# qingqing-zijin/LEAD-YOLO

Measured on AMD Instinct MI355X. Metric: images/sec (640x640) fwd+bwd, higher is better.
Workload: dtype bf16; 1 GPU; lead-yolo-s bs=64/gpu 3x640x640 bf16 full train step: uint8 batch -> train-mode forward (batch-statistics BN), ComputeLoss, HIP backward, clip 10, SGD-nesterov 3 groups, ModelEMA update (BASELINE.json configs[2]); random-init weights; global_batch=64, parallelism=dp1 (single GPU, no collective), world_size=1

## Files before the change

### include/lead_yolo_hip.h

```cpp
#ifndef LEAD_YOLO_HIP_H
#define LEAD_YOLO_HIP_H
#ifdef __cplusplus
extern "C" {
#endif

enum { LY_F32 = 0, LY_BF16 = 1 };
int ly_abi_version(void);
const char* ly_last_error(void);

int ly_mlpblock_fwd(const void* x , void* y , int n_img, int H, int W, int C, const void* wp, const void* w1,
                    const void* w2, const float* bn_scale, const float* bn_shift, double* stats, int dtype, void* stream);
int ly_mlpblock_pconv(const void* x , void* z , int n_img, int H, int W, int C, const void* wp, int dtype, void* stream);
int ly_mlpblock_bwd_ok(int C, int dtype);
long ly_mlpblock_bwd_slab_floats(int C);
int ly_mlpblock_bwd(const void* x , const void* dy , void* g , int n_img, int H, int W, int C, const void* wp, const void* w1,
                    const void* w2t, const void* w1t, const float* a, const float* b, const float* alpha, const float* kappa, const float* lambda,
                    double* stats, float* slab, long slab_floats, float* dw1, float* dw2, int pass, int dtype, void* stream);
int ly_mlpblock_bwd_dx_ok(int C, int W, int dtype);
int ly_mlpblock_bwd_dx(const void* g , const void* dy , const void* x , void* dx , int n_img, int H, int W, int C, const void* wpt,
                       float* slab, long slab_floats, float* dwp, int lddw, int dw_ts, int dw_cs, int dtype, void* stream);
int ly_mlpblock_hidden_tiles(int C);

enum { LY_ACT_NONE_ = 0, LY_ACT_RELU_ = 1, LY_ACT_SILU_ = 2 };
enum { LY_GATHER_ROWS = 0,
// ... 117 lines not shown
  float* dwc_part; int ng;
  int dtype;
} LyRf3cBwdParams;
int ly_rf3c_bwd(const LyRf3cBwdParams* p, int pass, void* stream);
int ly_rf3c_wgrad(const LyRf3cBwdParams* p, void* stream);


int ly_sppf_pool(const void* x , int ldx, int n_img, int H, int W, int C, int k, void* out , int ldo, int dtype, void* stream);
int ly_detect_tail(const void* y , int ldy, int n_img, int H, int W, int na, int no, const float* anchors, float stride,
                   float* p, float* z, long zrows, long zoff, int dtype, void* stream);
int ly_detect_level(const void* x , int ldx, int n_img, int H, int W, int K, const void* wp, int nat, const float* bias, int na, int no,
                    const float* anchors, float stride, float* p, float* z, long zrows, long zoff, int dtype, void* stream);
int ly_detect_level_ok(int K, int na, int no, int dtype);
int ly_detect_level_aug(const void* x , int ldx, int n_img, int H, int W, int K, const void* wp, int nat, const float* bias, int na, int no,
                        const float* anchors, float stride, float* p, float* z, long zrows, long zoff, float dscale, int dflip, float img_w,
                        int dtype, void* stream);
int ly_detect_tail_aug(const void* y , int ldy, int n_img, int H, int W, int na, int no, const float* anchors, float stride,
                       float* p, float* z, long zrows, long zoff, float dscale, int dflip, float img_w, int dtype, void* stream);

enum { LY_F16 = 2 };
#define LY_SCALE_IMG_MAX 4
typedef struct LyScaleImgSpec {
  void* out;
  int Hs, Ws;
  int Ho, Wo;
  int flip;
} LyScaleImgSpec;
int ly_scale_img(const void* x , int n_img, int C, int H, int W, const LyScaleImgSpec* specs, int nspec, float pad, int dtype, void* stream);

typedef struct LyMosaicTile {
  long off;
  int h, w;
  int x1a, y1a, x2a, y2a;
  int x1b, y1b;
  int lab, nlab;
  int src;
  int unused;
  double padw, padh;
} LyMosaicTile;
typedef struct LyMosaicImage {
  LyMosaicTile tile[4];
  double m[6];
  float minv[6];
  double scale;
  int mosaic;
  int flipud, fliplr;
  int unused;
  const unsigned char* lut;
} LyMosaicImage;
int ly_mosaic_img(const unsigned char* bank, const LyMosaicImage* imgs, int n_img, int s, unsigned char* out, void* stream);
int ly_mosaic_labels(const double* labels, const LyMosaicImage* imgs, int n_img, int s, int max_labels, float* targets, long cap, void* stream);
int ly_detect_head_bwd(const float* dp, int n_img, int H, int W, int na, int no, void* du , int ldu, float* dbias,
                       int dbias_f64 , int dtype, void* stream);


int ly_chan_moments(const void* x , int ldx, long rows, int C, double* mom , int dtype, void* stream);
int ly_coordatt_conv1_stats(const float* pool, long positions, int C, int mip, const float* w1, const float* b1,
                            double* stats , void* stream);
int ly_sum_rows_f64(const double* src, int R, int C, double* dst, void* stream);

int ly_rfcbam_tap_moments(const void* x , int ldx, int n_img, int H, int W, int C, int s, double* mom , int dtype, void* stream);
int ly_rfcbam_gen_prepare(const double* mom, int C, int k, const float* gen_w, const float* gamma, const float* beta, float eps,
                          float momentum, double count, float* running_mean, float* running_var, long* nbt, float* out8, float* a1,
                          float* wq_stats, float* wq_main, float* wq_c , int mom_stripes , void* stream);

int ly_nms_candidates(const float* pred, int bs, int N, int no, float conf_thres, unsigned long long class_mask, float* score, float* det,
                      void* stream);
int ly_nms_candidates_ml(const float* pred, int bs, int N, int no, float conf_thres, unsigned long long class_mask, float* score, float* det,
                         void* stream);
int ly_nms_greedy(const float* det, const long* order, const float* sorted_score, int bs, int N, float iou_thres, float max_wh, int max_det,
                  int max_nms, int* keep, int* count, void* stream);


int ly_bnact_fwd(const void* u , int ldu, long rows, int C, const float* a, const float* b, int act, void* y , int ldy, int dtype, void* stream);
int ly_bnact_bwd_reduce(const void* dy , int lddy, const void* u , int ldu, long rows, int C, const float* a, const float* b,
                        int act, double* sums , int dtype, void* stream);
int ly_bnact_bwd_apply(const void* dy , int lddy, const void* u , int ldu, long rows, int C, const float* a, const float* b,
                       int act, const float* alpha, const float* kappa, const float* lambda, void* du , int lddu, int dtype, void* stream);
int ly_bnact_bwd_reduce_pair(const void* dy1 , int lddy1, const void* dy2 , int lddy2, int csplit, const void* u , int ldu, long rows, int C,
                             const float* a, const float* b, int act, double* sums1, double* sums2, int dtype, void* stream);
int ly_bnact_bwd_apply_pair(const void* dy1 , int lddy1, const void* dy2 , int lddy2, int csplit, const void* u , int ldu, long rows, int C,
                            const float* a, const float* b, int act, const float* alpha, const float* kappa, const float* lambda, void* du , int lddu,
                            int dtype, void* stream);

typedef struct LyWgradParams {
  long M;
  int H, W;
  int N;
  const void* du; int lddu;
  const void* x; int ldx;
  int Hin, Win, Cin;
  int ks, stride, pad;
  int nchw, up2;
  float* dw; int lddw;
  int dtype;
  int dw_ts, dw_cs, n_valid, c_valid;
  const float* x_scale; const float* x_shift;
  float* ws; long ws_floats;
} LyWgradParams;
int ly_wgrad(const LyWgradParams* p, void* stream);
int ly_wgrad_group(const LyWgradParams* arr, int n, void* stream);
int ly_tune_wgrad3(int on);

int ly_up2_bwd(const void* d , int ldd, int n_img, int Hs, int Ws, int C, void* out , int ldo, int dtype, void* stream);
int ly_unpatch(const void* g , int n_img, int Ho, int Wo, int C, int ks, void* dx , int dtype, void* stream);
int ly_sum_rows(const float* src, long R, long C, long ld, float* dst, int accumulate, void* stream);
int ly_patch4_rows_u8(const unsigned char* img, int n_img, int C, int H, int W, void* rows , int dtype, void* stream);
int ly_patch4_wgrad_u8(const unsigned char* img, int n_img, int C, int H, int W, const void* du , int lddu, int N, float scale, float* slab,
                       long slab_floats, float* dw , int dtype, void* stream);

int ly_coordatt_gate_bwd(const void* dout , int ldd, const void* x , int ldx, int n_img, int H, int W, int C, const float* a_h,
                         const float* a_w, void* dx , int lddx, float* da_h, float* da_w, int bands, int slabs, int dtype, void* stream);
int ly_pool_hw_bwd(const float* gp, int n_img, int H, int W, int C, void* dx , int lddx, int accumulate, int dtype, void* stream);
int ly_maxpool_arg(const void* x , int ldx, int n_img, int H, int W, int C, int k, unsigned char* arg, int lda, int dtype, void* stream);
int ly_maxpool_gather(const unsigned char* arg, int lda, const float* d_up, int ldu, const void* d_own, int ldd, int own_dtype, int n_img, int H,
                      int W, int C, int k, void* out, int ldo, int out_dtype, void* stream);
int ly_sppf_bwd(const void* buf , int ldb, const void* d , int ldd, int n_img, int H, int W, int c, int k, void* out , int ldo, int dtype,
                void* stream);
int ly_mlp_dx(const void* dy , const void* g , const void* t , int ldt, long rows, int C, int c4, void* dx , int dtype, void* stream);
int ly_maxpool_bwd(const void* x , int ldx, const float* dy, int lddy, int n_img, int H, int W, int C, int k, float* dx, int lddx,
                   int dtype, void* stream);

int ly_rf_generate(const void* x , int ldx, int n_img, int H, int W, int C, int k, int s, const float* wg, void* ug , int dtype, void* stream);
int ly_rf_bwd_attn(int n_img, int H, int W, int C, int k, int s, const void* ug , const void* dcd , const float* ag, const float* bg,
                   const float* ca, const float* rfa, void* cd , float* d_rfa, float* gmax, float* d_ca, int dtype, void* stream);
int ly_rfa_bwd(const float* d_rfa, const float* rfa, const float* mm, const float* w18, int n_img, int Hk, int Wk, float* d_mm,
               float* dw18, int dw18_f64 , void* stream);
int ly_rf_bwd_relu(int n_img, int H, int W, int C, int k, int s, const void* ug , void* dcd , const float* ag, const float* bg,
                   const float* ca, const float* rfa, const float* gmax, const float* d_mm, float* sums, int dtype, void* stream);
int ly_rf_bwd_gen(const void* x , int ldx, int n_img, int H, int W, int C, int k, int s, const void* ug , void* dv , const float* alpha,
                  const float* kappa, const float* lambda, float* dwg, int part_rows, int dtype, void* stream);
int ly_rf_bwd_dx(int n_img, int H, int W, int C, int k, int s, const void* dug , const float* wg, void* dx , int lddx,
                 const float* addnc , float add_scale,
                 int dtype, void* stream);
int ly_se_bwd(const float* part, int slices, int n_img, int HW, int C, const float* wa, const float* wb, int R, const float* ca,
              const void* d_ca , int d_ca_f64, float* dwa, float* dwb,
              float* dgap, float* ws, void* stream);

#define LY_STATS_STRIPES 32
int ly_bn_finalize(const void* stats , int stats_f64, int stripes, int nch, int c_off, int N, double count, const float* gamma, const float* beta,
                   const float* bias, float eps, float momentum, float* running_mean, float* running_var, long* nbt, float* scale,
                   float* shift, float* mean, float* invstd, void* stream);
int ly_bn_bwd_coeffs(const void* sums , int sums_f64, int stripes, int N, double count, const float* a,
                     const float* mean, const float* invstd, int train, float* dgamma, float* dbeta, float* alpha, float* kappa, float* lambda,
                     int tr_a, int tr_b , void* stream);
int ly_bn_finalize_pair(const void* stats, int stats_f64, int stripes, int c_half, double count, const float* gamma0, const float* beta0, float eps0,
                        float momentum0, float* running_mean0, float* running_var0, long* nbt0, const float* gamma1, const float* beta1, float eps1,
                        float momentum1, float* running_mean1, float* running_var1, long* nbt1, float* scale, float* shift, float* mean,
                        float* invstd, void* stream);
int ly_bn_bwd_coeffs_pair(const void* sums0, const void* sums1, int sums_f64, int stripes, int c_half, double count, const float* a, const float* mean,
                          const float* invstd, float* dgamma0, float* dbeta0, float* dgamma1, float* dbeta1, float* alpha, float* kappa,
                          float* lambda, void* stream);
int ly_frag_pack3(const float* w, int R, int K, long ld_r, long ld_k, int rows_to, int planes, void* out, void* stream);

typedef struct LyPackDesc {
  const float* src; void* dst;
  int r_valid, K, planes, S, t0, T;
  int nrb, nb, nc, vb, vc;
  long sra, srb, sa, sb, sc;
  long blk0;
} LyPackDesc;
int ly_pack_table(const LyPackDesc* table, const int* blk_desc, int n_blocks, void* stream);

typedef struct LyRf1BwdParams {
  int n_img; long HW; int C;
  const void* x; int ldx;
// ... 64 lines not shown
```

### lead-yolo_amd/csrc/ly_attention.hip

```cpp
#include <float.h>

#include "ly_tile.hpp"
#include "ly_params.h"


template <typename T>
__global__ __launch_bounds__(LY_THREADS) void ly_pool_hw_kernel(const T* __restrict__ x, int ldx, int H, int W, int C,
                                                                 float* __restrict__ pool) {
  __shared__ f32x4 red[LY_THREADS];
  const int L = H + W;
  const int bid = ly_xcd_remap((int)blockIdx.x, (int)gridDim.x);
  const int n = bid / L, pos = bid - n * L;
  const int nc4 = C >> 2;
  const int tid = threadIdx.x;
  const int groups = LY_THREADS / nc4;
  const bool row = pos < H;
  const int len = row ? W : H;
  const long base = row ? ((long)n * H + pos) * W : ((long)n * H) * W + (pos - H);
  const long step = row ? 1 : W;
  const int c4 = tid % nc4, j0 = tid / nc4;
  f32x4 s = ly_zero4();
  if (j0 < groups) {
#pragma unroll 4
    for (int j = j0; j < len; j += groups) s += ly_ld4<T>(x + (base + j * step) * ldx + 4 * c4);
  }
  red[tid] = s;
  __syncthreads();
  if (j0 == 0) {
    for (int g = 1; g < groups; ++g) s += red[g * nc4 + c4];
    const float inv = 1.f / (float)len;
    ly_stg4(pool + ((long)n * L + pos) * C + 4 * c4, s * inv);
  }
}

extern "C" int ly_pool_hw(const void* x, int ldx, int n_img, int H, int W, int C, float* pool, int dtype, void* stream) {
  LY_CHECK_DTYPE(dtype, "pool_hw");
  LY_CHECK(x && pool && (C & 3) == 0 && (ldx & 3) == 0 && C <= 1024, "pool_hw: bad arguments (C=%d ldx=%d)", C, ldx);
  LY_WITH_T(dtype, hipLaunchKernelGGL(ly_pool_hw_kernel<T>, dim3(n_img * (H + W)), dim3(LY_THREADS), 0, reinterpret_cast<hipStream_t>(stream),
                                      reinterpret_cast<const T*>(x), ldx, H, W, C, pool));
  LY_LAUNCH_CHECK();
  return 0;
}

__global__ __launch_bounds__(LY_THREADS) void ly_coordatt_mlp_kernel(const float* __restrict__ pool, int H, int W, int C, int mip,
                                                                      const float* __restrict__ w1, const float* __restrict__ b1,
                                                                      const float* __restrict__ sc, const float* __restrict__ sh,
                                                                      const float* __restrict__ wh, const float* __restrict__ bh,
                                                                      const float* __restrict__ ww, const float* __restrict__ bw,
                                                                      float* __restrict__ a_h, float* __restrict__ a_w) {
  __shared__ float ys[64];
  const int L = H + W;
  const int n = blockIdx.x / L, pos = blockIdx.x - n * L;
  const int tid = threadIdx.x, lane = tid & 63, wave = tid >> 6;
  const float* p = pool + ((long)n * L + pos) * C;
  for (int m = wave; m < mip; m += 4) {
    float s = 0.f;
    for (int c = lane; c < C; c += 64) s += w1[m * C + c] * p[c];
    s = ly_group_sum(s, 64);
    if (lane == 0) ys[m] = ly_hswish(sc ? (s + b1[m]) * sc[m] + sh[m] : s + b1[m]);
  }
  __syncthreads();
  const bool isrow = pos < H;
  const float* wx = isrow ? wh : ww;
  const float* bx = isrow ? bh : bw;
  float* out = isrow ? a_h + ((long)n * H + pos) * C : a_w + ((long)n * W + (pos - H)) * C;
  for (int c = tid; c < C; c += LY_THREADS) {
    float s = bx[c];
    for (int m = 0; m < mip; ++m) s += wx[c * mip + m] * ys[m];
    out[c] = ly_sigmoid(s);
  }
}

extern "C" int ly_coordatt_mlp(const float* pool, int n_img, int H, int W, int C, int mip, const float* w1, const float* b1,
                               const float* sc, const float* sh, const float* wh, const float* bh, const float* ww, const float* bw, float* a_h, float* a_w,
                               void* stream) {
  LY_CHECK(pool && w1 && b1 && wh && bh && ww && bw && a_h && a_w && (!sc == !sh), "coordatt_mlp: null pointer");
  LY_CHECK(mip > 0 && mip <= 64, "coordatt_mlp: mip=%d out of range", mip);
  hipLaunchKernelGGL(ly_coordatt_mlp_kernel, dim3(n_img * (H + W)), dim3(LY_THREADS), 0, reinterpret_cast<hipStream_t>(stream),
                     pool, H, W, C, mip, w1, b1, sc, sh, wh, bh, ww, bw, a_h, a_w);
  LY_LAUNCH_CHECK();
  return 0;
}

template <typename T>
__global__ __launch_bounds__(LY_THREADS) void ly_colsum_kernel(const T* __restrict__ x, int ldx, int P, int C, int slices,
                                                                float* __restrict__ part) {
  __shared__ f32x4 red[LY_THREADS];
  const int n = blockIdx.x / slices, sl = blockIdx.x - n * slices;
  const int nc4 = C >> 2, tid = threadIdx.x;
  const int per = (P + slices - 1) / slices;
  const int j_lo = sl * per, j_hi = (j_lo + per) < P ? (j_lo + per) : P;
  const int groups = LY_THREADS / nc4;
  const int c4 = tid % nc4, j0 = tid / nc4;
  f32x4 s = ly_zero4();
  if (j0 < groups) {
#pragma unroll 4
    for (int j = j_lo + j0; j < j_hi; j += groups) s += ly_ld4<T>(x + ((long)n * P + j) * ldx + 4 * c4);
  }
  red[tid] = s;
  __syncthreads();
  if (j0 == 0) {
    for (int g = 1; g < groups; ++g) s += red[g * nc4 + c4];
    ly_stg4(part + ((long)n * slices + sl) * C + 4 * c4, s);
  }
}

__host__ __device__ __forceinline__ size_t ly_se_lds_floats(int C, int R) {
  const size_t base = (size_t)((C + R + 3) & ~3) + 4 * LY_THREADS;
  const size_t w = 2 * (size_t)R * C;
  return (C & 3) == 0 && w * 4 <= 48 * 1024 ? base + w : base;
}

__device__ __forceinline__ void ly_se_mlp_body(float* sm, const int n, const float* __restrict__ part, int slices, int C, float inv_hw,
                                               const float* __restrict__ wa, const float* __restrict__ wb, int R, float* __restrict__ ca) {
  float* g = sm;
  float* hid = sm + C;
  f32x4* red = reinterpret_cast<f32x4*>(sm + ((C + R + 3) & ~3));
  const size_t base = (size_t)((C + R + 3) & ~3) + 4 * LY_THREADS;
  const bool staged = ly_se_lds_floats(C, R) > base;
  float* was = sm + base;
  float* wbs = was + (size_t)R * C;
  const int tid = threadIdx.x, lane = tid & 63, wave = tid >> 6;
// ... 1544 lines not shown
```

### lead-yolo_amd/csrc/ly_backward.hip

```cpp
#include "ly_tile.hpp"
#include "ly_params.h"

template <int ACT>
__device__ __forceinline__ f32x4 ly_dact4(const f32x4 v, const f32x4 dy) {
  f32x4 r;
#pragma unroll
  for (int i = 0; i < 4; ++i) {
    if (ACT == LY_ACT_RELU) {
      r[i] = v[i] > 0.f ? dy[i] : 0.f;
    } else if (ACT == LY_ACT_SILU) {
      const float s = ly_sigmoid(v[i]);
      r[i] = dy[i] * s * (1.f + v[i] * (1.f - s));
    } else {
      r[i] = dy[i];
    }
  }
  return r;
}

#ifndef LY_XCD_STREAM
#define LY_XCD_STREAM 1
#endif
#if LY_XCD_STREAM
#define LY_XCD_RANGE(total)                                                                                             \
  const bool xr_on = gridDim.x >= 8;                           \
  const long xr_x = blockIdx.x & 7, xr_slot = blockIdx.x >> 3, xr_n = ((long)gridDim.x + 7 - xr_x) >> 3;                  \
  const long xr_per = (((total) + 7) / 8 + LY_THREADS - 1) / LY_THREADS * LY_THREADS;                                      \
  const long xr_lo = xr_x * xr_per, xr_hi = xr_lo + xr_per < (total) ? xr_lo + xr_per : (total);                           \
  const long xr_begin = xr_on ? xr_lo + xr_slot * LY_THREADS + threadIdx.x : (long)blockIdx.x * LY_THREADS + threadIdx.x; \
  const long xr_end = xr_on ? xr_hi : (total), xr_step = (xr_on ? xr_n : (long)gridDim.x) * LY_THREADS
#else
#define LY_XCD_RANGE(total)                                                                                             \
  const long xr_begin = (long)blockIdx.x * LY_THREADS + threadIdx.x, xr_end = (total), xr_step = (long)gridDim.x * LY_THREADS
#endif

#define LY_EW_UR 4
#define LY_XCD_ROWS(rows_, groups_)                                                                                     \
  const bool xw_on = gridDim.x >= 8;                                                                                      \
  const long xw_x = blockIdx.x & 7, xw_slot = blockIdx.x >> 3, xw_n = ((long)gridDim.x + 7 - xw_x) >> 3;                  \
  const long xw_per = ((rows_) + 7) / 8;                                                                                  \
  const long xw_lo = xw_on ? xw_x * xw_per : 0, xw_end = xw_on ? (xw_lo + xw_per < (rows_) ? xw_lo + xw_per : (rows_)) : (rows_); \
  const long xw_begin = xw_lo + (xw_on ? xw_slot : (long)blockIdx.x) * (groups_);                                         \
  const long xw_step = (xw_on ? xw_n : (long)gridDim.x) * (groups_)

template <typename T, int ACT>
__global__ __launch_bounds__(LY_THREADS) void ly_bnact_bwd_reduce_kernel(const T* __restrict__ dy, int lddy, const T* __restrict__ u,
                                                                          int ldu, long rows, int C, const float* __restrict__ a,
                                                                          const float* __restrict__ b, double* __restrict__ sums,
                                                                          const T* __restrict__ dy2, int lddy2, int csplit, double* __restrict__ sums2) {
  __shared__ f32x4 red1[LY_THREADS], red2[LY_THREADS];
  using R4 = typename LyT<T>::R4;
  const int ncv = C >> 2, tid = threadIdx.x;
  const int groups = LY_THREADS / ncv;
  const int cv = tid % ncv, j0 = tid / ncv;
  f32x4 s1 = ly_zero4(), s2 = ly_zero4();
  const bool second = 4 * cv >= csplit;
  if (j0 < groups) {
    const f32x4 av = ly_ldg4(a + 4 * cv), bv = ly_ldg4(b + 4 * cv);
    constexpr int UR = 4;
    LY_XCD_ROWS(rows, groups);
    const long stride = xw_step;
    const T* const dyb = second ? dy2 + (4 * cv - csplit) : dy + 4 * cv;
    const long ldd = second ? lddy2 : lddy;
    for (long r0 = xw_begin + j0; r0 < xw_end; r0 += UR * stride) {
      R4 qu[UR], qg[UR];
#pragma unroll
      for (int k = 0; k < UR; ++k) {
        const long r = r0 + k * stride < xw_end ? r0 + k * stride : xw_end - 1;
        qu[k] = ly_ldr4<T>(u + r * ldu + 4 * cv);
        qg[k] = ly_ldr4<T>(dyb + r * ldd);
      }
#pragma unroll
      for (int k = 0; k < UR; ++k) {
        const f32x4 uu = ly_r4_f32(qu[k]);
        f32x4 dv = ly_dact4<ACT>(av * uu + bv, ly_r4_f32(qg[k]));
        if (!(r0 + k * stride < xw_end)) dv = ly_zero4();
        s1 += dv;
        s2 += dv * uu;
      }
    }
  }
  red1[tid] = s1;
  red2[tid] = s2;
  __syncthreads();
  if (j0 == 0) {
    const int ch = second ? C - csplit : csplit, lc = 4 * cv - (second ? csplit : 0);
    double* sm = (second ? sums2 : sums) + (size_t)(blockIdx.x & (LY_STATS_STRIPES - 1)) * 2 * ch;
    for (int g = 1; g < groups; ++g) { s1 += red1[g * ncv + cv]; s2 += red2[g * ncv + cv]; }
#pragma unroll
    for (int r = 0; r < 4; ++r) {
      atomicAdd(sm + lc + r, (double)s1[r]);
      atomicAdd(sm + ch + lc + r, (double)s2[r]);
    }
  }
}

template <typename T, int ACT>
__global__ __launch_bounds__(LY_THREADS) void ly_bnact_bwd_apply_kernel(const T* __restrict__ dy, int lddy, const T* u, int ldu,
                                                                         long rows, int C, const float* __restrict__ a,
                                                                         const float* __restrict__ b, const float* __restrict__ alpha,
                                                                         const float* __restrict__ kappa, const float* __restrict__ lambda,
                                                                         T* du, int lddu, const T* __restrict__ dy2, int lddy2, int csplit) {
  constexpr int VW = LyT<T>::VW, NQ = VW / 4;
  using RV = typename LyT<T>::RV;
  if ((C % VW) == 0 && (ldu % VW) == 0 && (lddy % VW) == 0 && (lddu % VW) == 0 && (lddy2 % VW) == 0 && (csplit % VW) == 0 && C / VW <= LY_THREADS) {
    const int ncv = C / VW, groups = LY_THREADS / ncv;
    const int cv = threadIdx.x % ncv, j0 = threadIdx.x / ncv;
    if (j0 >= groups) return;
    const int c = VW * cv;
    f32x4 ca[NQ], cb[NQ], cal[NQ], cka[NQ], cla[NQ];
#pragma unroll
    for (int q = 0; q < NQ; ++q) {
      ca[q] = ly_ldg4(a + c + 4 * q); cb[q] = ly_ldg4(b + c + 4 * q);
      cal[q] = ly_ldg4(alpha + c + 4 * q); cka[q] = ly_ldg4(kappa + c + 4 * q); cla[q] = ly_ldg4(lambda + c + 4 * q);
    }
    LY_XCD_ROWS(rows, groups);
    const T* const gb = c >= csplit ? dy2 + (c - csplit) : dy + c;
    const long ldg = c >= csplit ? lddy2 : lddy;
    for (long r0 = xw_begin + j0; r0 < xw_end; r0 += LY_EW_UR * xw_step) {
      RV qu[LY_EW_UR], qg[LY_EW_UR];
#pragma unroll
      for (int k = 0; k < LY_EW_UR; ++k) {
        const long r = r0 + k * xw_step < xw_end ? r0 + k * xw_step : xw_end - 1;
        qu[k] = ly_ldrv<T>(u + r * ldu + c);
        qg[k] = ly_ldrv<T>(gb + r * ldg);
      }
#pragma unroll
      for (int k = 0; k < LY_EW_UR; ++k) {
        f32x4 uu[NQ], g[NQ];
        ly_rv_unpack(qu[k], uu);
        ly_rv_unpack(qg[k], g);
#pragma unroll
        for (int q = 0; q < NQ; ++q) {
          const f32x4 dv = ly_dact4<ACT>(ca[q] * uu[q] + cb[q], g[q]);
          uu[q] = cal[q] * dv + cka[q] + cla[q] * uu[q];
        }
        const long r = r0 + k * xw_step;
        if (r < xw_end) *reinterpret_cast<RV*>(du + r * lddu + c) = ly_rv_pack(uu, (RV*)nullptr);
      }
    }
    return;
  }
  const int nc4 = C >> 2;
  const long total = rows * nc4;
  LY_XCD_RANGE(total);
  for (long i = xr_begin; i < xr_end; i += xr_step) {
    const long r = i / nc4;
    const int c = 4 * (int)(i - r * nc4);
    const f32x4 uu = ly_ld4<T>(u + r * ldu + c);
    const f32x4 g = ly_ld4<T>(c >= csplit ? dy2 + r * lddy2 + (c - csplit) : dy + r * lddy + c);
    const f32x4 dv = ly_dact4<ACT>(ly_ldg4(a + c) * uu + ly_ldg4(b + c), g);
    ly_st4<T>(du + r * lddu + c, ly_ldg4(alpha + c) * dv + ly_ldg4(kappa + c) + ly_ldg4(lambda + c) * uu);
  }
}

template <typename T, int ACT>
__global__ __launch_bounds__(LY_THREADS) void ly_bnact_fwd_kernel(const T* __restrict__ u, int ldu, long rows, int C, const float* __restrict__ a,
                                                                   const float* __restrict__ b, T* __restrict__ y, int ldy) {
  constexpr int VW = LyT<T>::VW, NQ = VW / 4;
  using RV = typename LyT<T>::RV;
  if ((C % VW) == 0 && (ldu % VW) == 0 && (ldy % VW) == 0 && C / VW <= LY_THREADS) {
    const int ncv = C / VW, groups = LY_THREADS / ncv;
    const int cv = threadIdx.x % ncv, j0 = threadIdx.x / ncv;
    if (j0 >= groups) return;
    const int c = VW * cv;
    f32x4 ca[NQ], cb[NQ];
#pragma unroll
    for (int q = 0; q < NQ; ++q) { ca[q] = ly_ldg4(a + c + 4 * q); cb[q] = ly_ldg4(b + c + 4 * q); }
    LY_XCD_ROWS(rows, groups);
    for (long r0 = xw_begin + j0; r0 < xw_end; r0 += LY_EW_UR * xw_step) {
      RV qu[LY_EW_UR];
#pragma unroll
      for (int k = 0; k < LY_EW_UR; ++k) {
        const long r = r0 + k * xw_step < xw_end ? r0 + k * xw_step : xw_end - 1;
        qu[k] = ly_ldrv<T>(u + r * ldu + c);
      }
#pragma unroll
      for (int k = 0; k < LY_EW_UR; ++k) {
        f32x4 uu[NQ];
        ly_rv_unpack(qu[k], uu);
#pragma unroll
        for (int q = 0; q < NQ; ++q) uu[q] = ly_act4(ca[q] * uu[q] + cb[q], ACT);
        const long r = r0 + k * xw_step;
        if (r < xw_end) *reinterpret_cast<RV*>(y + r * ldy + c) = ly_rv_pack(uu, (RV*)nullptr);
      }
    }
    return;
  }
  const int nc4 = C >> 2;
  const long total = rows * nc4;
  LY_XCD_RANGE(total);
  for (long i = xr_begin; i < xr_end; i += xr_step) {
    const long r = i / nc4;
    const int c = 4 * (int)(i - r * nc4);
    const f32x4 v = ly_ldg4(a + c) * ly_ld4<T>(u + r * ldu + c) + ly_ldg4(b + c);
    ly_st4<T>(y + r * ldy + c, ly_act4(v, ACT));
  }
}

static long ly_ew_blocks(long items) {
  long b = (items + LY_THREADS * 4L - 1) / (LY_THREADS * 4L);
  return b < 1 ? 1 : b > 4096 ? 4096 : b;
}
static long ly_ew_row_blocks(long rows, int C, int vw) {
  const int ncv = C / vw;
  if (ncv <= 0 || ncv > LY_THREADS) return ly_ew_blocks(rows * (C >> 2));
  const long groups = LY_THREADS / ncv;
  const long trips = ((rows + 7) / 8 + groups * LY_EW_UR - 1) / (groups * LY_EW_UR);
  const long per = (trips + 255) / 256;
  const long bx = (trips + per - 1) / per;
  return 8 * (bx < 1 ? 1 : bx);
}

extern "C" int ly_bnact_fwd(const void* u_, int ldu, long rows, int C, const float* a, const float* b, int act, void* y_, int ldy, int dtype, void* stream) {
  LY_CHECK_DTYPE(dtype, "bnact_fwd");
  LY_CHECK(u_ && a && b && y_ && rows > 0, "bnact_fwd: null pointer");
  LY_CHECK((C & 3) == 0 && C > 0 && (ldu & 3) == 0 && (ldy & 3) == 0, "bnact_fwd: C=%d / ld must be multiples of 4", C);
  const int vw_ = dtype == LY_BF16 ? 8 : 4;
  const bool vec_ = (C % vw_) == 0 && (ldu % vw_) == 0 && (ldy % vw_) == 0 && C / vw_ <= LY_THREADS;
  const long blocks = vec_ ? ly_ew_row_blocks(rows, C, vw_) : ly_ew_blocks(rows * (C >> 2));
  hipStream_t st = reinterpret_cast<hipStream_t>(stream);
  LY_WITH_T(dtype, {
    const T* u = reinterpret_cast<const T*>(u_);
    T* y = reinterpret_cast<T*>(y_);
    if (act == LY_ACT_SILU) hipLaunchKernelGGL((ly_bnact_fwd_kernel<T, LY_ACT_SILU>), dim3((unsigned)blocks), dim3(LY_THREADS), 0, st, u, ldu, rows, C, a, b, y, ldy);
    else if (act == LY_ACT_RELU) hipLaunchKernelGGL((ly_bnact_fwd_kernel<T, LY_ACT_RELU>), dim3((unsigned)blocks), dim3(LY_THREADS), 0, st, u, ldu, rows, C, a, b, y, ldy);
    else hipLaunchKernelGGL((ly_bnact_fwd_kernel<T, LY_ACT_NONE>), dim3((unsigned)blocks), dim3(LY_THREADS), 0, st, u, ldu, rows, C, a, b, y, ldy);
  });
  LY_LAUNCH_CHECK();
  return 0;
}

static int bnact_bwd_reduce_launch(const void* dy_, int lddy, const void* dy2_, int lddy2, int csplit, const void* u_, int ldu, long rows, int C, const float* a,
                                   const float* b, int act, double* sums, double* sums2, int dtype, void* stream) {
  const int vw = 4;
  const int groups = LY_THREADS / (C / vw);
#ifndef LY_RED_ROWS
#define LY_RED_ROWS 32
#endif
  long blocks = (rows + groups * (long)LY_RED_ROWS - 1) / (groups * (long)LY_RED_ROWS);
  blocks = blocks < 1 ? 1 : blocks > 2048 ? 2048 : blocks;
  if (blocks >= 8) blocks = (blocks + 7) / 8 * 8;
  hipStream_t st = reinterpret_cast<hipStream_t>(stream);
#define LY_RED(A) hipLaunchKernelGGL((ly_bnact_bwd_reduce_kernel<T, A>), dim3((unsigned)blocks), dim3(LY_THREADS), 0, st, dy, lddy, u, ldu, rows, C, a, b, sums, dy2, lddy2, csplit, sums2)
  LY_WITH_T(dtype, {
    const T* dy = reinterpret_cast<const T*>(dy_);
    const T* dy2 = reinterpret_cast<const T*>(dy2_);
    const T* u = reinterpret_cast<const T*>(u_);
    if (act == LY_ACT_SILU) LY_RED(LY_ACT_SILU);
    else if (act == LY_ACT_RELU) LY_RED(LY_ACT_RELU);
    else LY_RED(LY_ACT_NONE);
  });
#undef LY_RED
  LY_LAUNCH_CHECK();
  return 0;
}

extern "C" int ly_bnact_bwd_reduce(const void* dy_, int lddy, const void* u_, int ldu, long rows, int C, const float* a, const float* b,
                                   int act, double* sums, int dtype, void* stream) {
  LY_CHECK_DTYPE(dtype, "bnact_bwd_reduce");
  LY_CHECK(dy_ && u_ && a && b && sums && rows > 0, "bnact_bwd_reduce: null pointer");
  LY_CHECK((C & 3) == 0 && C > 0 && C <= 1024 && (lddy & 3) == 0 && (ldu & 3) == 0, "bnact_bwd_reduce: C=%d / ld must be multiples of 4", C);
  return bnact_bwd_reduce_launch(dy_, lddy, dy_, lddy, C, u_, ldu, rows, C, a, b, act, sums, sums, dtype, stream);
}

extern "C" int ly_bnact_bwd_reduce_pair(const void* dy1, int lddy1, const void* dy2, int lddy2, int csplit, const void* u_, int ldu, long rows, int C,
                                        const float* a, const float* b, int act, double* sums1, double* sums2, int dtype, void* stream) {
  LY_CHECK_DTYPE(dtype, "bnact_bwd_reduce_pair");
  LY_CHECK(dy1 && dy2 && u_ && a && b && sums1 && sums2 && rows > 0, "bnact_bwd_reduce_pair: null pointer");
  LY_CHECK((C & 3) == 0 && C > 0 && C <= 1024 && csplit > 0 && csplit < C && (csplit & 3) == 0 && (lddy1 & 3) == 0 && (lddy2 & 3) == 0 && (ldu & 3) == 0,
           "bnact_bwd_reduce_pair: C=%d csplit=%d / ld must be multiples of 4", C, csplit);
  return bnact_bwd_reduce_launch(dy1, lddy1, dy2, lddy2, csplit, u_, ldu, rows, C, a, b, act, sums1, sums2, dtype, stream);
}

static int bnact_bwd_apply_launch(const void* dy_, int lddy, const void* dy2_, int lddy2, int csplit, const void* u_, int ldu, long rows, int C, const float* a,
                                  const float* b, int act, const float* alpha, const float* kappa, const float* lambda, void* du_, int lddu, int dtype, void* stream) {
  const int vw_ = dtype == LY_BF16 ? 8 : 4;
  const bool vec_ = (C % vw_) == 0 && (ldu % vw_) == 0 && (lddy % vw_) == 0 && (lddu % vw_) == 0 && (lddy2 % vw_) == 0 && (csplit % vw_) == 0 && C / vw_ <= LY_THREADS;
  const long blocks = vec_ ? ly_ew_row_blocks(rows, C, vw_) : ly_ew_blocks(rows * (C >> 2));
  hipStream_t st = reinterpret_cast<hipStream_t>(stream);
#define LY_APP(A) hipLaunchKernelGGL((ly_bnact_bwd_apply_kernel<T, A>), dim3((unsigned)blocks), dim3(LY_THREADS), 0, st, dy, lddy, u, ldu, rows, C, a, b, alpha, kappa, lambda, du, lddu, dy2, lddy2, csplit)
  LY_WITH_T(dtype, {
    const T* dy = reinterpret_cast<const T*>(dy_);
    const T* dy2 = reinterpret_cast<const T*>(dy2_);
    const T* u = reinterpret_cast<const T*>(u_);
    T* du = reinterpret_cast<T*>(du_);
    if (act == LY_ACT_SILU) LY_APP(LY_ACT_SILU);
    else if (act == LY_ACT_RELU) LY_APP(LY_ACT_RELU);
    else LY_APP(LY_ACT_NONE);
  });
#undef LY_APP
  LY_LAUNCH_CHECK();
  return 0;
}

extern "C" int ly_bnact_bwd_apply(const void* dy_, int lddy, const void* u_, int ldu, long rows, int C, const float* a, const float* b,
                                  int act, const float* alpha, const float* kappa, const float* lambda, void* du_, int lddu, int dtype, void* stream) {
  LY_CHECK_DTYPE(dtype, "bnact_bwd_apply");
  LY_CHECK(dy_ && u_ && a && b && alpha && kappa && lambda && du_ && rows > 0, "bnact_bwd_apply: null pointer");
  LY_CHECK((C & 3) == 0 && C > 0 && (lddy & 3) == 0 && (ldu & 3) == 0 && (lddu & 3) == 0, "bnact_bwd_apply: C=%d / ld must be multiples of 4", C);
  return bnact_bwd_apply_launch(dy_, lddy, dy_, lddy, C, u_, ldu, rows, C, a, b, act, alpha, kappa, lambda, du_, lddu, dtype, stream);
}

extern "C" int ly_bnact_bwd_apply_pair(const void* dy1, int lddy1, const void* dy2, int lddy2, int csplit, const void* u_, int ldu, long rows, int C,
                                       const float* a, const float* b, int act, const float* alpha, const float* kappa, const float* lambda, void* du_,
                                       int lddu, int dtype, void* stream) {
  LY_CHECK_DTYPE(dtype, "bnact_bwd_apply_pair");
  LY_CHECK(dy1 && dy2 && u_ && a && b && alpha && kappa && lambda && du_ && rows > 0, "bnact_bwd_apply_pair: null pointer");
  LY_CHECK((C & 3) == 0 && C > 0 && csplit > 0 && csplit < C && (csplit & 3) == 0 && (lddy1 & 3) == 0 && (lddy2 & 3) == 0 && (ldu & 3) == 0 && (lddu & 3) == 0,
           "bnact_bwd_apply_pair: C=%d csplit=%d / ld must be multiples of 4", C, csplit);
  return bnact_bwd_apply_launch(dy1, lddy1, dy2, lddy2, csplit, u_, ldu, rows, C, a, b, act, alpha, kappa, lambda, du_, lddu, dtype, stream);
}

__device__ __forceinline__ void ly_split8(const float (&v)[8], bf16x8& hi, bf16x8& lo) {
  bf16x4 h0, l0, h1, l1;
  ly_split4((f32x4){v[0], v[1], v[2], v[3]}, h0, l0);
  ly_split4((f32x4){v[4], v[5], v[6], v[7]}, h1, l1);
  hi = ly_cat8(h0, h1);
  lo = ly_cat8(l0, l1);
}

template <typename T, bool ROWS>
__global__ __launch_bounds__(LY_THREADS) void ly_wgrad_kernel(const LyWgradParams P, const int tiles_k, const long chunk_px) {
  constexpr int PL = LyT<T>::PL;
  const T* const du = reinterpret_cast<const T*>(P.du);
  const T* const xin = reinterpret_cast<const T*>(P.x);
  const int tid = threadIdx.x, lane = tid & 63;
  const int wave = __builtin_amdgcn_readfirstlane(tid >> 6);
  const int li = lane & 15, lq = lane >> 4;
  const int tk = blockIdx.x % tiles_k, tn = blockIdx.x / tiles_k;
  const int n_base = tn * 64 + (wave & 1) * 32, k_base = tk * 64 + (wave >> 1) * 32;
  const long p_begin = (long)blockIdx.y * chunk_px;
  const long p_end = p_begin + chunk_px < P.M ? p_begin + chunk_px : P.M;
  const int Ktot = P.ks * P.ks * P.Cin;

  int arow[2], bcol[2], ky[2], kx[2], cc[2];
  bool aok[2], bok[2];
#pragma unroll
  for (int t = 0; t < 2; ++t) {
    const int r = n_base + 16 * t + li;
    aok[t] = r < P.N;
    arow[t] = aok[t] ? r : 0;
    const int c = k_base + 16 * t + li;
    bok[t] = c < Ktot;
    bcol[t] = bok[t] ? c : 0;
    const int tap = bcol[t] / P.Cin;
    cc[t] = bcol[t] - tap * P.Cin;
    ky[t] = tap / P.ks;
    kx[t] = tap - ky[t] * P.ks;
  }
  const int Hv = P.up2 ? 2 * P.Hin : P.Hin, Wv = P.up2 ? 2 * P.Win : P.Win;
  const float invW = 1.f / (float)P.W, invH = 1.f / (float)P.H;

  f32x4 acc[2][2];
#pragma unroll
  for (int i = 0; i < 2; ++i)
#pragma unroll
    for (int j = 0; j < 2; ++j) acc[i][j] = ly_zero4();

  for (long p0 = p_begin; p0 < p_end; p0 += 32) {
    float av[2][8], bv[2][8];
    const long pf = p0 + 8 * lq;
    int n_i = 0, ho = 0, wo = 0;
    if (!ROWS) {
      const int g = (int)(pf < P.M ? pf : P.M - 1);
      const int row = ly_fdiv(g, P.W, invW);
      wo = g - row * P.W;
      n_i = ly_fdiv(row, P.H, invH);
      ho = row - n_i * P.H;
    }
#pragma unroll
    for (int j = 0; j < 8; ++j) {
      const long p = pf + j;
      const bool pok = p < p_end;
      const long pc = pok ? p : p_end - 1;
#pragma unroll
      for (int t = 0; t < 2; ++t) {
        const float v = ly_ld1<T>(du + pc * P.lddu + arow[t]);
        av[t][j] = (pok && aok[t]) ? v : 0.f;
      }
      if (ROWS) {
#pragma unroll
        for (int t = 0; t < 2; ++t) {
          const float v = ly_ld1<T>(xin + pc * P.ldx + bcol[t]);
          bv[t][j] = (pok && bok[t]) ? v : 0.f;
        }
      } else {
#pragma unroll
        for (int t = 0; t < 2; ++t) {
          int hi = ho * P.stride + ky[t] - P.pad, wi = wo * P.stride + kx[t] - P.pad;
          const bool ok = pok && bok[t] && hi >= 0 && hi < Hv && wi >= 0 && wi < Wv;
          if (P.up2) { hi >>= 1; wi >>= 1; }
          long off = P.nchw ? (((long)n_i * P.Cin + cc[t]) * P.Hin + hi) * P.Win + wi
                            : (((long)n_i * P.Hin + hi) * P.Win + wi) * P.ldx + cc[t];
          const float v = ly_ld1<T>(xin + (ok ? off : 0));
// ... 1660 lines not shown
```

### lead-yolo_amd/csrc/ly_tile.hpp

```cpp
#pragma once
#include "ly_common.hpp"
#include "ly_params.h"

typedef __bf16 bf16x8 __attribute__((ext_vector_type(8)));
typedef __bf16 bf16x4 __attribute__((ext_vector_type(4)));
typedef __bf16 bf16x2 __attribute__((ext_vector_type(2)));
typedef float f32x2 __attribute__((ext_vector_type(2)));

typedef unsigned int ly_u32x2 __attribute__((ext_vector_type(2)));
typedef unsigned int ly_u32x4 __attribute__((ext_vector_type(4)));
template <typename T> struct LyT;
template <> struct LyT<float> {
  static constexpr int PL = 2, VW = 4;
  static constexpr bool BF = false;
  typedef f32x4 R4;
  typedef f32x4 RV;
};
template <> struct LyT<__bf16> {
  static constexpr int PL = 1, VW = 8;
  static constexpr bool BF = true;
  typedef ly_u32x2 R4;
  typedef ly_u32x4 RV;
};
template <> struct LyT<unsigned char> {
  static constexpr int PL = 2, VW = 4;
  static constexpr bool BF = false;
  typedef unsigned R4;
  typedef unsigned RV;
};

struct ly_bf16img { unsigned short v; };
struct ly_f16img { unsigned short v; };
struct ly_h4raw { ly_u32x2 r; };
template <> struct LyT<ly_bf16img> {
  static constexpr int PL = 2, VW = 4;
  static constexpr bool BF = false;
  typedef ly_u32x2 R4;
  typedef ly_u32x2 RV;
};
template <> struct LyT<ly_f16img> {
  static constexpr int PL = 2, VW = 4;
  static constexpr bool BF = false;
  typedef ly_h4raw R4;
  typedef ly_h4raw RV;
};

#define LY_WITH_T(dtype, ...)                                 \
  do {                                                        \
    if ((dtype) == LY_BF16) { using T = __bf16; __VA_ARGS__; } \
    else { using T = float; __VA_ARGS__; }                    \
  } while (0)
#define LY_CHECK_DTYPE(dtype, who) LY_CHECK((dtype) == LY_F32 || (dtype) == LY_BF16, who ": unknown dtype %d", (dtype))

__device__ __forceinline__ f32x4 ly_cvt4(const bf16x4 h) { return __builtin_convertvector(h, f32x4); }
__device__ __forceinline__ bf16x4 ly_cvtb4(const f32x4 v) { return __builtin_convertvector(v, bf16x4); }

template <typename T> __device__ __forceinline__ f32x4 ly_ld4(const T* p);
template <> __device__ __forceinline__ f32x4 ly_ld4<float>(const float* p) { return *reinterpret_cast<const f32x4*>(p); }
template <> __device__ __forceinline__ f32x4 ly_ld4<__bf16>(const __bf16* p) { return ly_cvt4(*reinterpret_cast<const bf16x4*>(p)); }
template <typename T> __device__ __forceinline__ void ly_st4(T* p, const f32x4 v);
template <> __device__ __forceinline__ void ly_st4<float>(float* p, const f32x4 v) { *reinterpret_cast<f32x4*>(p) = v; }
template <> __device__ __forceinline__ void ly_st4<__bf16>(__bf16* p, const f32x4 v) { *reinterpret_cast<bf16x4*>(p) = ly_cvtb4(v); }
template <typename T> __device__ __forceinline__ float ly_ld1(const T* p) { return (float)*p; }
template <typename T> __device__ __forceinline__ void ly_st1(T* p, float v) { *p = (T)v; }

template <typename T> __device__ __forceinline__ typename LyT<T>::R4 ly_ldr4(const T* p) { return *reinterpret_cast<const typename LyT<T>::R4*>(p); }
template <typename T> __device__ __forceinline__ typename LyT<T>::RV ly_ldrv(const T* p) { return *reinterpret_cast<const typename LyT<T>::RV*>(p); }
__device__ __forceinline__ f32x4 ly_r4_f32(const f32x4 r) { return r; }
__device__ __forceinline__ f32x4 ly_r4_f32(const ly_u32x2 r) { return ly_cvt4(__builtin_bit_cast(bf16x4, r)); }
__device__ __forceinline__ void ly_zero_raw(f32x4& r) { r = (f32x4){0.f, 0.f, 0.f, 0.f}; }
__device__ __forceinline__ void ly_zero_raw(ly_u32x2& r) { r = (ly_u32x2){0u, 0u}; }
__device__ __forceinline__ void ly_zero_raw(ly_u32x4& r) { r = (ly_u32x4){0u, 0u, 0u, 0u}; }
__device__ __forceinline__ void ly_zero_raw(unsigned& r) { r = 0u; }
__device__ __forceinline__ void ly_zero_raw(ly_h4raw& r) { r.r = (ly_u32x2){0u, 0u}; }
__device__ __forceinline__ f32x4 ly_u8x4_f32(unsigned r) {
  return (f32x4){(float)(r & 255u), (float)((r >> 8) & 255u), (float)((r >> 16) & 255u), (float)(r >> 24)} * (1.f / 255.f);
}
__device__ __forceinline__ void ly_rv_unpack(const f32x4 r, f32x4 (&q)[1]) { q[0] = r; }
__device__ __forceinline__ void ly_rv_unpack(const ly_u32x4 r, f32x4 (&q)[2]) {
  const bf16x8 b = __builtin_bit_cast(bf16x8, r);
  q[0] = ly_cvt4(__builtin_shufflevector(b, b, 0, 1, 2, 3));
  q[1] = ly_cvt4(__builtin_shufflevector(b, b, 4, 5, 6, 7));
}
__device__ __forceinline__ f32x4 ly_rv_pack(const f32x4 (&q)[1], f32x4*) { return q[0]; }
__device__ __forceinline__ ly_u32x4 ly_rv_pack(const f32x4 (&q)[2], ly_u32x4*) {
  const bf16x4 a = ly_cvtb4(q[0]), b = ly_cvtb4(q[1]);
  return __builtin_bit_cast(ly_u32x4, __builtin_shufflevector(a, b, 0, 1, 2, 3, 4, 5, 6, 7));
}

__device__ __forceinline__ void ly_split4(const f32x4 v, bf16x4& hi, bf16x4& lo) {
  hi = __builtin_convertvector(v, bf16x4);
  const f32x4 back = __builtin_convertvector(hi, f32x4);
  lo = __builtin_convertvector(v - back, bf16x4);
}

__device__ __forceinline__ bf16x8 ly_cat8(const bf16x4 a, const bf16x4 b) {
  return __builtin_shufflevector(a, b, 0, 1, 2, 3, 4, 5, 6, 7);
}

__device__ __forceinline__ f32x4 ly_mfma_bf16(const bf16x8 a, const bf16x8 b, f32x4 c) {
  return __builtin_amdgcn_mfma_f32_16x16x32_bf16(a, b, c, 0, 0, 0);
}

__device__ __forceinline__ f32x4 ly_mfma3(const bf16x8 whi, const bf16x8 wlo, const bf16x8 xhi, const bf16x8 xlo, f32x4 acc) {
  acc = ly_mfma_bf16(whi, xlo, acc);
  acc = ly_mfma_bf16(wlo, xhi, acc);
  acc = ly_mfma_bf16(whi, xhi, acc);
  return acc;
}

__host__ __device__ constexpr int ly_kp(int k) { return (k + 31) / 32 * 32; }
__host__ __device__ constexpr int ly_rs(int kp) { return 2 * kp + 16; }

__device__ __forceinline__ void ly_lds_put4(char* hi_plane, char* lo_plane, int row_byte, int c, const f32x4 v) {
  bf16x4 h, l;
  ly_split4(v, h, l);
  *reinterpret_cast<bf16x4*>(hi_plane + row_byte + 2 * c) = h;
  *reinterpret_cast<bf16x4*>(lo_plane + row_byte + 2 * c) = l;
}

__device__ __forceinline__ void ly_lds_put_r4(char* hi_plane, char* lo_plane, int row_byte, int c, const f32x4 v) { ly_lds_put4(hi_plane, lo_plane, row_byte, c, v); }
__device__ __forceinline__ void ly_lds_put_r4(char* hi_plane, char*, int row_byte, int c, const ly_u32x2 v) {
  *reinterpret_cast<ly_u32x2*>(hi_plane + row_byte + 2 * c) = v;
}
__device__ __forceinline__ void ly_lds_put_rv(char* hi_plane, char* lo_plane, int row_byte, int c, const f32x4 v) { ly_lds_put4(hi_plane, lo_plane, row_byte, c, v); }
__device__ __forceinline__ void ly_lds_put_rv(char* hi_plane, char*, int row_byte, int c, const ly_u32x4 v) {
  *reinterpret_cast<ly_u32x4*>(hi_plane + row_byte + 2 * c) = v;
}
__device__ __forceinline__ void ly_lds_put_rv(char* hi_plane, char* lo_plane, int row_byte, int c, const unsigned v) { ly_lds_put4(hi_plane, lo_plane, row_byte, c, ly_u8x4_f32(v)); }
__device__ __forceinline__ void ly_lds_put_rv(char* hi_plane, char* lo_plane, int row_byte, int c, const ly_u32x2 v) {
  ly_lds_put4(hi_plane, lo_plane, row_byte, c, ly_cvt4(__builtin_bit_cast(bf16x4, v)));
}
typedef _Float16 ly_f16x4 __attribute__((ext_vector_type(4)));
__device__ __forceinline__ void ly_lds_put_rv(char* hi_plane, char* lo_plane, int row_byte, int c, const ly_h4raw v) {
  ly_lds_put4(hi_plane, lo_plane, row_byte, c, __builtin_convertvector(__builtin_bit_cast(ly_f16x4, v.r), f32x4));
}
template <int PL>
__device__ __forceinline__ void ly_lds_put_f32(char* hi_plane, char* lo_plane, int row_byte, int c, const f32x4 v) {
  if constexpr (PL == 2) ly_lds_put4(hi_plane, lo_plane, row_byte, c, v);
  else *reinterpret_cast<bf16x4*>(hi_plane + row_byte + 2 * c) = ly_cvtb4(v);
}

__device__ __forceinline__ bf16x8 ly_lds_frag(const char* plane, int row_byte, int s, int lq) {
  const char* p = plane + row_byte + 2 * (32 * s + 4 * lq);
  const bf16x4 a = *reinterpret_cast<const bf16x4*>(p);
// ... 93 lines not shown
```

### lead-yolo_amd/grad.py

```python
import ctypes

import os

import torch

from . import ops, pack
from .ops import ACT_NONE, ACT_RELU, ACT_SILU


def _rows_dense(t):
    t = ops.nhwc(t)
    if t.stride(1) != 1:
        t = t.permute(0, 2, 3, 1).contiguous().permute(0, 3, 1, 2)
    return t




FORK_SUM = True


class _Slot:
    __slots__ = ("deferred",)

    def __init__(self):
        self.deferred = []


class Fork(torch.autograd.Function):
    @staticmethod
    def forward(ctx, x, slot):
        ctx.slot = slot
        ctx.set_materialize_grads(False)
        return x.view_as(x), x.view_as(x)

    @staticmethod
    def backward(ctx, d1, d2):
        total = d1 if d2 is None else d2 if d1 is None else d1 + d2
        deferred, ctx.slot.deferred = ctx.slot.deferred, []
        with torch.no_grad():
            for produce in deferred:
                total = produce(total)
        return total, None


def fork(x):
    slot = _Slot()
    a, b = Fork.apply(x, slot)
    a._ly_slot = b._ly_slot = slot
    return a, b


def _slot_of(x):
    return getattr(x, "_ly_slot", None) if (FORK_SUM and x is not None) else None


def _gemm_dx(slot, n, c, h, w, like, **kw):
    def produce(eadd):
        out = ops.empty_nhwc(n, c, h, w, like)
        extra, late = {}, None
        if eadd is not None:
            if eadd.dtype == out.dtype and tuple(eadd.shape) == tuple(out.shape) and kw["N"] % 4 == 0:
                e, lde = ops.rows(eadd)
                extra = dict(eadd=e, ldeadd=lde)
            else:
                late = eadd
        ops.gemm(out=out, **kw, **extra)
        return out if late is None else out + late.to(out.dtype)
    if slot is None:
        return produce(None)
    slot.deferred.append(produce)
    return None


class ConvSpec:

    def __init__(self, kind, cout, act=ACT_NONE, bn=None, bn_train=False, k=1, nchw=False, up=False, out_dtype=None):
        self.kind = kind
        self.cout, self.act, self.bn, self.bn_train = cout, act, bn, bn_train
        self.k, self.nchw, self.up = k, nchw, up
        self.out_dtype = out_dtype




def _conv_forward(spec, x0, x1, wp, e_scale, e_shift, act, stats=None, out=None, store=False):
    co = spec.cout
    if spec.kind == "pw":
        t0, ld0 = ops.rows(x0)
        n, c0, h, w = t0.shape
        if spec.up:
            h, w = 2 * h, 2 * w
        kw = dict(a0=t0, lda0=ld0, k0=c0, gather=ops.GATHER_UP2 if spec.up else ops.GATHER_ROWS)
        k = c0
        if x1 is not None:
            t1, ld1 = ops.rows(x1)
            kw.update(a1=t1, lda1=ld1)
            k += t1.shape[1]
        if (stats is None or store) and out is None:
            out = ops.empty_nhwc(n, co, h, w, t0)
        ops.gemm(M=n * h * w, H=h, W=w, K=k, N=co, wp=wp, out=out, ldo=co, e_scale=e_scale, e_shift=e_shift, act=act, stats=stats, **kw)
        return out
    if spec.kind == "c3":
        t0, ld0 = ops.rows(x0)
        n, c, h, w = t0.shape
        if (stats is None or store) and out is None:
            out = ops.empty_nhwc(n, co, h, w, t0)
        ops.conv3x3(M=n * h * w, H=h, W=w, Cin=c, N=co, x=t0, ldx=ld0, wp=wp, out=out, ldo=co, e_scale=e_scale, e_shift=e_shift, act=act,
                    stats=stats)
        return out
    n, c, h, w = x0.shape
    k = spec.k
    ho, wo = h // k, w // k
    if spec.nchw:
        xr = x0.contiguous()
        kw = dict(K=16 * c, a0=xr, lda0=0, k0=16 * c, gather=ops.GATHER_PATCH_NCHW, Hin=h, Win=w, Cin=c, ks=4, pk=0)
    else:
        xr = _rows_dense(x0)
        kw = dict(K=k * k * c, a0=xr, lda0=c, k0=k * k * c, gather=ops.GATHER_PATCH, Hin=h, Win=w, Cin=c, ks=k, pk=k * c)
    odt = spec.out_dtype or xr.dtype
    if (stats is None or store) and out is None:
        out = ops.empty_nhwc(n, co, ho, wo, xr, dtype=odt)
    ops.gemm(M=n * ho * wo, H=ho, W=wo, N=co, wp=wp, out=out, ldo=co, e_scale=e_scale, e_shift=e_shift, act=act, stats=stats, dtype=odt, **kw)
    return out




def affine_backward(dy, u, a, b, act, mean, invstd, train, inplace=True, gamma=None, beta=None, lddy=None, out=None):
    n, c, h, w = u.shape
    rows = n * h * w
    lddy = c if lddy is None else lddy
    sums = ops.bnact_bwd_reduce(dy, lddy, u, c, rows, c, a, b, act)
    tg, tb = ops.grad_target(gamma), ops.grad_target(beta)
    direct = tg is not None and tb is not None and tg.numel() == c and tb.numel() == c
    dgamma, dbeta, alpha, kappa, lam = ops.bn_bwd_coeffs(sums, c, rows, a, mean, invstd, train, dgamma=tg if direct else None,
                                                         dbeta=tb if direct else None)
    if direct:
        ops.grad_done(gamma)
        ops.grad_done(beta)
    du = out if out is not None else u if inplace else torch.empty_like(u)
    ops.bnact_bwd_apply(dy, lddy, u, c, rows, c, a, b, act, alpha, kappa, lam, du, c)
    return du, dgamma, dbeta


def conv_wgrad(spec, du, x0, x1, weight):
    n, co, ho, wo = du.shape
    m = n * ho * wo
    nv = weight.shape[0]
    tgt = ops.grad_target(weight)
    dw = tgt if tgt is not None else torch.zeros(weight.shape, dtype=torch.float32, device=du.device)
    if spec.kind == "pw":
        t0, ld0 = ops.rows(x0)
        c0 = t0.shape[1]
        k = c0 + (x1.shape[1] if x1 is not None else 0)
        probs = [dict(M=m, H=ho, W=wo, N=co, du=du, lddu=co, x=t0, ldx=ld0, Hin=t0.shape[2], Win=t0.shape[3], Cin=c0, dw=dw, lddw=k,
                      up2=spec.up, n_valid=nv)]
        if x1 is not None:
            t1, ld1 = ops.rows(x1)
            probs.append(dict(M=m, H=ho, W=wo, N=co, du=du, lddu=co, x=t1, ldx=ld1, Hin=ho, Win=wo, Cin=t1.shape[1], dw=dw, lddw=k, dw_off=c0,
                              n_valid=nv))
        ops.wgrad_group(probs)
    elif spec.kind == "c3":
        t0, ld0 = ops.rows(x0)
        c = t0.shape[1]
        ts, cs = (c, 1) if _tap_major(dw) else (1, 9)
        ops.wgrad(M=m, H=ho, W=wo, N=co, du=du, lddu=co, x=t0, ldx=ld0, Hin=ho, Win=wo, Cin=c, dw=dw, lddw=9 * c, ks=3, stride=1, pad=1,
                  dw_ts=ts, dw_cs=cs, n_valid=nv)
    else:
        _, c, h, w = x0.shape
        k = spec.k
        if spec.nchw and h == ho * k and w == wo * k and (k * k * c) % 4 == 0 and co % 4 == 0:
            u8 = x0.dtype == torch.uint8
            if u8 and k == 4 and co == nv and dw.is_contiguous() and ops.patch4_wgrad_u8_ok(x0, du, co):
                ops.patch4_wgrad_u8(x0, du, co, co, dw, 1.0 / 255.0)
                if tgt is not None:
                    ops.grad_done(weight)
                    return None
                return dw
            if u8 and k == 4 and x0.is_contiguous():
                xr = ops.patch4_rows_u8(x0, du.dtype)
            else:
                xr = x0.reshape(n, c, ho, k, wo, k).permute(0, 2, 4, 1, 3, 5).reshape(m, c * k * k).to(du.dtype)
            acc = ops.zeros_f32(weight.numel(), du.device).view(weight.shape) if u8 else dw
            ops.wgrad(M=m, H=ho, W=wo, N=co, du=du, lddu=co, x=xr, ldx=k * k * c, Hin=ho, Win=wo, Cin=k * k * c, dw=acc, lddw=k * k * c, n_valid=nv)
            if u8:
                dw.add_(acc, alpha=1.0 / 255.0)
        elif spec.nchw:
            if x0.dtype == torch.uint8:
                raise NotImplementedError("uint8 image: the weight gradient of the patch embedding needs H, W multiples of the patch size")
            xr = x0.contiguous().to(du.dtype)
            ops.wgrad(M=m, H=ho, W=wo, N=co, du=du, lddu=co, x=xr, ldx=0, Hin=h, Win=w, Cin=c, dw=dw, lddw=k * k * c, ks=k, stride=k, nchw=True,
                      dw_ts=1, dw_cs=k * k, n_valid=nv)
        else:
            xr = _rows_dense(x0)
            ts, cs = (c, 1) if _tap_major(dw) else (1, k * k)
            ops.wgrad(M=m, H=ho, W=wo, N=co, du=du, lddu=co, x=xr, ldx=c, Hin=h, Win=w, Cin=c, dw=dw, lddw=k * k * c, ks=k, stride=k,
                      dw_ts=ts, dw_cs=cs, n_valid=nv)
    if tgt is not None:
        ops.grad_done(weight)
        return None
    return dw


def _tap_major_rows(g):
    if g is None or not _tap_major(g):
        return None
    co, ci, kh, kw = g.shape
    rows = g.permute(0, 2, 3, 1)
    if not rows.is_contiguous():
        return None
    return rows.view(co, kh * kw * ci)


def _tap_major(g):
    return g.dim() == 4 and not g.is_contiguous() and g.stride(1) == 1 and g.stride(3) == g.shape[1]


def conv_dgrad(spec, du, weight, x0, x1, need0, need1, slots=(None, None)):
    n, co, ho, wo = du.shape
    m = n * ho * wo
    with torch.no_grad():
        if spec.kind == "pw":
            nw, kin = weight.shape[0], weight.numel() // weight.shape[0]
            wt = pack.packed(pack.src_matrix(weight, kin, nw, sr=1, sk=kin, k_pad=co), co, ops.planes_of(du))
            if x1 is None and not spec.up and slots[0] is not None and kin % 4 == 0:
                return _gemm_dx(slots[0], n, kin, ho, wo, du, M=m, H=ho, W=wo, K=co, N=kin, a0=du, lda0=co, k0=co, wp=wt, ldo=kin), None
            d = ops.empty_nhwc(n, kin, ho, wo, du)
            ops.gemm(M=m, H=ho, W=wo, K=co, N=kin, a0=du, lda0=co, k0=co, wp=wt, out=d, ldo=kin)
            if x1 is None:
                return (ops.up2_bwd(d, kin, n, ho // 2, wo // 2, kin) if spec.up else d), None
            c0 = x0.shape[1]
            d0 = d[:, :c0]
            if spec.up and need0:
                d0 = ops.up2_bwd(d, kin, n, ho // 2, wo // 2, c0)
            return (d0 if need0 else None), (d[:, c0:] if need1 else None)
        if spec.kind == "c3":
            cop = (weight.shape[0] + 31) // 32 * 32
            wt = pack.packed(pack.src_taps(weight, cop, transposed_flipped=True), 9 * cop, ops.planes_of(du))
            cin = weight.shape[1]
            d = ops.empty_nhwc(n, cin, ho, wo, du)
            ops.conv3x3(M=m, H=ho, W=wo, Cin=co, N=cin, x=du, ldx=co, wp=wt, out=d, ldo=cin)
            return d, None
        if spec.nchw:
            raise NotImplementedError("gradient with respect to the NCHW input image is not built (never needed: it is the data)")
        _, c, h, w = x0.shape
        k = spec.k
        wt = pack.packed(pack.Src(weight, k * k * c, nrb=c, sra=1, srb=k * k, nc=co, sc=c * k * k), co, ops.planes_of(du))
        if h == ho * k and w == wo * k and c % 4 == 0:
            return _gemm_dx(slots[0], n, c, h, w, du, M=m, H=ho, W=wo, K=co, N=k * k * c, a0=du, lda0=co, k0=co, wp=wt, ldo=c, scat_ks=k,
                            scat_c=c), None
        g = torch.empty((m, k * k * c), dtype=du.dtype, device=du.device)
        ops.gemm(M=m, H=ho, W=wo, K=co, N=k * k * c, a0=du, lda0=co, k0=co, wp=wt, out=g, ldo=k * k * c)
        return ops.unpatch(g, n, ho, wo, c, k, h, w), None


def _pad_cols(w2d, k):
    if w2d.shape[1] == k:
        return w2d
    out = torch.zeros(w2d.shape[0], k, dtype=w2d.dtype, device=w2d.device)
    out[:, :w2d.shape[1]] = w2d
    return out


class ConvBnAct(torch.autograd.Function):

    @staticmethod
    def forward(ctx, spec, wp, x0, x1, weight, bias, gamma, beta):
        co = spec.cout
        dev = x0.device
        ctx.slots = (_slot_of(x0), _slot_of(x1))
        bias_f = bias.detach().float().contiguous() if bias is not None else None
        mean = invstd = None
        if spec.bn is not None:
            if spec.bn_train and co % 4 == 0:
                stats = ops.new_stats(co, dev)
                u = _conv_forward(spec, x0, x1, wp, None, bias_f, ACT_NONE, stats=stats, store=True)
                rows = u.shape[0] * u.shape[2] * u.shape[3]
                a, b, mean, invstd = ops.bn_finalize(spec.bn, stats, co, rows, want_stats=True)
                y = torch.empty_like(u)
                ops.bnact_fwd(u, co, rows, co, a, b, spec.act, y, co)
                ctx.spec, ctx.wp = spec, wp
                ctx.has = (x1 is not None, bias is not None)
                ctx.params = (weight, gamma, beta)
                ctx.save_for_backward(x0, x1, weight, bias_f, a, b, mean, invstd, u)
                return y
            elif spec.bn_train:
                stats = ops.new_stats(co, dev)
                _conv_forward(spec, x0, x1, wp, None, bias_f, ACT_NONE, stats=stats)
                y0 = _out_shape(spec, x0)
                a, b, mean, invstd = ops.bn_finalize(spec.bn, stats, co, y0[0] * y0[2] * y0[3], want_stats=True)
            else:
                bn = spec.bn
                invstd = torch.rsqrt(bn.running_var.detach().float() + bn.eps)
                mean = bn.running_mean.detach().float()
                a = (gamma.detach().float() * invstd).contiguous()
                b = (beta.detach().float() - mean * a).contiguous()
            sh = b if bias_f is None else (b + bias_f * a).contiguous()
            y = _conv_forward(spec, x0, x1, wp, a, sh, spec.act)
        else:
            a = b = None
            y = _conv_forward(spec, x0, x1, wp, None, bias_f, spec.act)
        ctx.spec, ctx.wp = spec, wp
        ctx.has = (x1 is not None, bias is not None)
        ctx.params = (weight, gamma, beta)
        ctx.save_for_backward(x0, x1, weight, bias_f, a, b, mean, invstd, None)
        return y

    @staticmethod
    def backward(ctx, dy):
        spec, wp = ctx.spec, ctx.wp
        x0, x1, weight, bias_f, a, b, mean, invstd, u_saved = ctx.saved_tensors
        w_param, g_param, b_param = ctx.params
        co = spec.cout
        need = ctx.needs_input_grad
        with torch.no_grad():
            odt = spec.out_dtype or x0.dtype
            dy = dy if dy.dtype == odt else dy.to(odt)
            lddy = None
            if spec.bn is not None or spec.act != ACT_NONE:
                dy, lddy = ops.rows(dy)
            else:
                dy = _rows_dense(dy)
            dgamma = dbeta = dbias = None
            if spec.bn is not None or spec.act != ACT_NONE:
                u = u_saved if u_saved is not None else _conv_forward(spec, x0, x1, wp, None, bias_f, ACT_NONE)
                if spec.bn is None:
                    a = torch.ones(co, dtype=torch.float32, device=dy.device)
                    b = torch.zeros_like(a)
                    mean, invstd = b, a
                du, dgamma, dbeta = affine_backward(dy, u, a, b, spec.act, mean, invstd, spec.bn is not None and spec.bn_train,
                                                    inplace=u_saved is None, gamma=g_param if spec.bn is not None else None,
                                                    beta=b_param if spec.bn is not None else None, lddy=lddy)
                if bias_f is not None:
                    if spec.bn is None:
                        dbias, dgamma, dbeta = dbeta, None, None
                    elif spec.bn_train:
                        dbias = torch.zeros_like(bias_f)
                    else:
                        dbias = a * (dbeta if dbeta is not None else b_param.grad)
                elif spec.bn is None:
                    dgamma = dbeta = None
            else:
                du = dy
                if bias_f is not None:
                    n, _, h, w = dy.shape
                    dbias = _chan_sum(dy, co)
            vw = ops.vw_of(du)
            cq = (co + vw - 1) // vw * vw
            if cq != co:
                n, _, h, w = du.shape
                pad = torch.zeros((n, cq, h, w), dtype=du.dtype, device=du.device).contiguous(memory_format=torch.channels_last)
                pad[:, :co] = du
                du_d = pad
            else:
                du_d = du
            dw = conv_wgrad(spec, du_d if spec.kind == "pw" else du, x0, x1, w_param) if need[4] else None
            dx0 = dx1 = None
            if need[2] or need[3]:
                dspec = spec
                if cq != co:
                    dspec = ConvSpec(spec.kind, cq, k=spec.k, nchw=spec.nchw, up=spec.up)
                dx0, dx1 = conv_dgrad(dspec, du_d, weight, x0, x1, need[2], need[3], ctx.slots)
        return None, None, dx0, dx1, dw, dbias, dgamma, dbeta


def _chan_sum(t, c):
    n, _, h, w = t.shape
    if c % 4 == 0 and c <= 1024:
        return ops.chan_moments(t, c, n * h * w, c)[:c]
    return t.sum((0, 2, 3), dtype=torch.float32)


def _out_shape(spec, x0):
    n, c, h, w = x0.shape
    if spec.kind == "patch":
        return n, spec.cout, h // spec.k, w // spec.k
    if spec.up:
        return n, spec.cout, 2 * h, 2 * w
    return n, spec.cout, h, w


def conv_bn_act(spec, wp, x0, x1, weight, bias, bn):
    gamma = bn.weight if bn is not None else None
    beta = bn.bias if bn is not None else None
    return ConvBnAct.apply(spec, wp, x0, x1, weight, bias, gamma, beta)


class ConvBnActPair(torch.autograd.Function):

    @staticmethod
    def forward(ctx, spec, wp, bn1, bn2, x0, x1, w1, w2, g1, be1, g2, be2):
        co = spec.cout
        c_ = co // 2
        stats = ops.new_stats(co, x0.device)
        u = _conv_forward(spec, x0, x1, wp, None, None, ACT_NONE, stats=stats, store=True)
        rows = u.shape[0] * u.shape[2] * u.shape[3]
        v = torch.empty(4, co, dtype=torch.float32, device=x0.device)
        ops.bn_finalize_pair(bn1, bn2, stats, c_, rows, v)
        y = torch.empty_like(u)
        ops.bnact_fwd(u, co, rows, co, v[0], v[1], spec.act, y, co)
        ctx.spec = spec
        ctx.wt_src = pack.src_matrix_kcat_t(w1, w2)
        ctx.slots = (_slot_of(x0), _slot_of(x1))
        ctx.split = spec.up or (x1 is not None and (ctx.slots[0] is not None or ctx.slots[1] is not None))
        if ctx.split:
            c0 = x0.shape[1]
            ctx.wt_src = (pack.src_matrix_kcat_t(w1, w2, 0, c0), pack.src_matrix_kcat_t(w1, w2, c0, None) if x1 is not None else None)
        ctx.params = ((w1, g1, be1), (w2, g2, be2))
        ctx.save_for_backward(x0, x1, w1, w2, v, u)
        return y[:, :c_], y[:, c_:]

    @staticmethod
    def backward(ctx, dy1, dy2):
        spec = ctx.spec
        x0, x1, w1, w2, v, u = ctx.saved_tensors
# ... 223 lines not shown
                       x_scale=a if pro else None, x_shift=b if pro else None)
            du1, dgamma, dbeta = affine_backward(dh, u1, a, b, ACT_RELU, mean, invstd, True, gamma=p_gamma, beta=p_beta, out=dh if pro else None)
            g = ops.empty_nhwc(n, c, h, w, x)
            ops.gemm(M=m, H=h, W=w, K=2 * c, N=c, a0=du1, lda0=2 * c, k0=2 * c, wp=pack.packed(pack.src_matrix(p_w1, c, 2 * c, sr=1, sk=c), 2 * c, pl), out=g, ldo=c)
            dw1, d1 = sink(p_w1)
            ops.wgrad_group([wg2, dict(M=m, H=h, W=w, N=2 * c, du=du1, lddu=2 * c, x=z, ldx=c, Hin=h, Win=w, Cin=c, dw=dw1, lddw=c)])
            dwp, dp = sink(p_wpc)
            ts, cs = (c4, 1) if _tap_major(dwp) else (1, 9)
            ops.wgrad(M=m, H=h, W=w, N=c4p, du=g, lddu=c, x=x, ldx=c, Hin=h, Win=w, Cin=c4p, dw=dwp, lddw=9 * c4, ks=3, stride=1, pad=1,
                      dw_ts=ts, dw_cs=cs, n_valid=c4, c_valid=c4)
            dx = torch.empty_like(dy)
            gz = torch.empty_like(g)
            if ops.mlpblock_bwd_dx_ok(x, c, w):
                dx, _ = ops.mlpblock_bwd_dx(g, dy, x, n, h, w, c, pack.packed(pack.src_taps(p_wpc, c4p, transposed_flipped=True), 9 * c4p, pl))
            elif ops.mlpblock_pconv(g, gz, n, h, w, c, pack.packed(pack.src_taps(p_wpc, c4p, transposed_flipped=True), 9 * c4p, pl)):
                _lib().check(_lib().lib().ly_mlp_dx(_lib().ptr(dy), _lib().ptr(gz), _lib().ptr(gz), c, m, c, 4, _lib().ptr(dx), _lib().dtype_code(dy),
                                                    _lib().stream_ptr()), "ly_mlp_dx")
            else:
                t = ops.empty_nhwc(n, c4p, h, w, x)
                wt = pack.packed(pack.src_taps(p_wpc, c4q, transposed_flipped=True), 9 * c4q, pl)
                ops.conv3x3(M=m, H=h, W=w, Cin=c4p, N=c4, x=g, ldx=c, wp=wt, out=t, ldo=c4p)
                _lib().check(_lib().lib().ly_mlp_dx(_lib().ptr(dy), _lib().ptr(g), _lib().ptr(t), c4p, m, c, c4, _lib().ptr(dx), _lib().dtype_code(dy),
                                                    _lib().stream_ptr()), "ly_mlp_dx")
            for prm, direct in ((p_wpc, dp), (p_w1, d1), (p_w2, d2)):
                if direct:
                    ops.grad_done(prm)
        return (None, dx, None if dp else dwp, None if d1 else dw1, dgamma, dbeta, None if d2 else dw2)


def _mlpblock_backward_fused(ctx, dy):
    x, wpc, w1, w2, a, b, mean, invstd = ctx.saved_tensors
    p_wpc, p_w1, p_gamma, p_beta, p_w2 = ctx.params
    n, c, h, w = x.shape
    m = n * h * w
    c4 = c // 4
    c4p = _ceil4(c4)
    pl = ops.planes_of(x)
    htp = (2 * c // 16 + 1) // 2 * 2
    pk_p, pk_1, _ = ctx.mod._weights(pl)
    pk_2t = pack.packed(pack.src_matrix(p_w2, 2 * c, c, sr=1, sk=2 * c), c, pl, rows_to=16 * htp)
    pk_1t = pack.packed(pack.src_matrix(p_w1, c, 2 * c, sr=1, sk=c), 2 * c, pl)
    sums = ops.new_stats(2 * c, x.device)
    ops.mlpblock_bwd(x, dy, n, h, w, c, pk_p, pk_1, pk_2t, pk_1t, a, b, stats=sums)
    tg, tb = ops.grad_target(p_gamma), ops.grad_target(p_beta)
    direct = tg is not None and tb is not None and tg.numel() == 2 * c and tb.numel() == 2 * c
    dgamma, dbeta, alpha, kappa, lam = ops.bn_bwd_coeffs(sums, 2 * c, m, a, mean, invstd, True, dgamma=tg if direct else None,
                                                         dbeta=tb if direct else None)
    if direct:
        ops.grad_done(p_gamma)
        ops.grad_done(p_beta)

    def sink(p):
        t = ops.grad_target(p)
        return (t, True) if t is not None and t.is_contiguous() else (torch.zeros(p.shape, dtype=torch.float32, device=x.device), False)
    dw1, d1 = sink(p_w1)
    dw2, d2 = sink(p_w2)
    g = ops.empty_nhwc(n, c, h, w, x)
    ops.mlpblock_bwd(x, dy, n, h, w, c, pk_p, pk_1, pk_2t, pk_1t, a, b, g=g, alpha=alpha, kappa=kappa, lam=lam, dw1=dw1, dw2=dw2)
    tgt = ops.grad_target(p_wpc)
    dwp, dp = (tgt, True) if tgt is not None else (torch.zeros(p_wpc.shape, dtype=torch.float32, device=x.device), False)
    ts, cs = (c4, 1) if _tap_major(dwp) else (1, 9)
    wt = pack.packed(pack.src_taps(p_wpc, c4p, transposed_flipped=True), 9 * c4p, pl)
    dx, wdone = ops.mlpblock_bwd_dx(g, dy, x, n, h, w, c, wt, dwp=dwp, lddw=9 * c4, dw_ts=ts, dw_cs=cs)
    if not wdone:
        ops.wgrad(M=m, H=h, W=w, N=c4p, du=g, lddu=c, x=x, ldx=c, Hin=h, Win=w, Cin=c4p, dw=dwp, lddw=9 * c4, ks=3, stride=1, pad=1,
                  dw_ts=ts, dw_cs=cs, n_valid=c4, c_valid=c4)
    for prm, direct_ in ((p_wpc, dp), (p_w1, d1), (p_w2, d2)):
        if direct_:
            ops.grad_done(prm)
    return (None, dx, None if dp else dwp, None if d1 else dw1, dgamma, dbeta, None if d2 else dw2)


MlpBlockFn._backward_fused = staticmethod(_mlpblock_backward_fused)


class CoordAttFn(torch.autograd.Function):

    @staticmethod
    def forward(ctx, mod, x, w1, b1, gamma, beta, wh, bh, ww, bw):
        t, ld = ops.rows(x)
        n, c, h, w = t.shape
        mip = mod.mip
        W1, Wh, Ww = (p.detach().reshape(p.shape[0], -1) for p in (w1, wh, ww))
        pool = ops.pool_hw(t, ld, n, h, w, c)
        st = ops.coordatt_conv1_stats(pool, n * (h + w), c, mip, W1, b1)
        sc, sh, mean, invstd = ops.bn_finalize(mod.bn1, st.view(1, -1), mip, n * (h + w), want_stats=True)
        a_h, a_w = ops.coordatt_mlp(pool, n, h, w, c, mip, W1, b1.detach(), Wh, bh.detach(), Ww, bw.detach(), sc=sc, sh=sh)
        out = ops.coordatt_gate(t, ld, n, h, w, c, a_h, a_w)
        ctx.save_for_backward(t, pool, a_h, a_w, mean, invstd)
        ctx.params = (w1, b1, gamma, beta, wh, bh, ww, bw)
        ctx.mip = mip
        return out

    @staticmethod
    def backward(ctx, dout):
        t, pool, a_h, a_w, mean, invstd = ctx.saved_tensors
        xr, ld = ops.rows(t)
        n, c, h, w = xr.shape
        w1, b1, gamma, beta, wh, bh, ww, bw = ctx.params
        dr, ldd = ops.rows(dout if dout.dtype == xr.dtype else dout.to(xr.dtype))
        dx, da_h, da_w = ops.coordatt_gate_bwd(dr, xr, ld, n, h, w, c, a_h, a_w, ldd=ldd)
        targets, ret = [], []
        for i, p in enumerate(ctx.params):
            if i == 1:
                sunk = p.requires_grad and ops.grad_target(p) is not None
                ret.append(None if (sunk or not p.requires_grad) else torch.zeros_like(p))
                continue
            tgt = ops.grad_target(p) if p.requires_grad else None
            fresh = tgt is None
            if fresh:
                tgt = torch.zeros(p.shape, dtype=torch.float32, device=xr.device)
            targets.append(tgt)
            ret.append(tgt if (fresh and p.requires_grad) else None)
        defer = ops.small_grads_ok() and all(r is None for r in ret) and all(t.is_contiguous() for t in targets)
        no_sink = all(q is None or not q.requires_grad or ops.grad_target(q) is None for i, q in enumerate(ctx.params) if i != 1)
        fresh64 = (not defer) and ops.DETERMINISTIC_SMALL_GRADS and no_sink
        if defer:
            targets = [ops.small_grad_scratch(t, q) for t, q in zip(targets, [q for i, q in enumerate(ctx.params) if i != 1])]
        elif fresh64:
            shapes = [t.shape for t in targets]
            targets = [ops.zeros_f64(t.numel(), xr.device) for t in targets]
        W1, Wh, Ww = (p.detach().reshape(p.shape[0], -1) for p in (w1, wh, ww))
        dpool = ops.coordatt_mlp_bwd(pool, n, h, w, c, ctx.mip, W1, b1.detach(), mean, invstd, gamma.detach(), beta.detach(), Wh, Ww, a_h, a_w,
                                     da_h, da_w, targets)
        if fresh64:
            rounded, k, out = ops.f64_round(targets, shapes), 0, []
            for i, r in enumerate(ret):
                if i == 1:
                    out.append(r)
                    continue
                out.append(rounded[k] if r is not None else None)
                k += 1
            ret = out
        ops.pool_hw_bwd(dpool, n, h, w, c, into=dx)
        for i, (p, r) in enumerate(zip(ctx.params, ret)):
            if r is None and p.requires_grad and not (defer and i != 1):
                ops.grad_done(p)
        return (None, dx, *ret)


def coordatt_train(mod, x):
    n, c, h, w = x.shape
    params = (mod.conv1.weight, mod.conv1.bias, mod.bn1.weight, mod.bn1.bias, mod.conv_h.weight, mod.conv_h.bias, mod.conv_w.weight, mod.conv_w.bias)
    if mod.mip in (8, 16) and c <= 512 and all(p is not None and p.dtype == torch.float32 for p in params):
        return CoordAttFn.apply(mod, x, *params)
    raise NotImplementedError(f"CoordAtt training is built for mip = max(8, c // 32) in (8, 16) and c <= 512 with float32 parameters (got mip={mod.mip}, "
                              f"c={c}): ly_coordatt_mlp_bwd has no instantiation for other widths, and there is no ATen fallback on the hot path")


class SppfPool(torch.autograd.Function):
    @staticmethod
    def forward(ctx, y, k):
        t, ld = ops.rows(y)
        n, c, h, w = t.shape
        if not ops.sppf_pool_fits(h, w):
            raise NotImplementedError("SPPF training path needs the map to fit the LDS pooling kernel")
        buf = ops.empty_nhwc(n, 4 * c, h, w, t)
        ops.sppf_pool(t, ld, n, h, w, c, k, buf, 4 * c)
        ctx.save_for_backward(buf)
        ctx.k = k
        return buf

    @staticmethod
    def backward(ctx, d):
        buf, = ctx.saved_tensors
        n, c4, h, w = buf.shape
        c = c4 // 4
        k = ctx.k
        if k != 5 or c % 4 != 0:
            acc = _rows_dense(d).float() if d.dtype != torch.float32 else _rows_dense(d).clone()
            for j in (2, 1, 0):
                ops.maxpool_bwd(buf, j * c, c4, acc, (j + 1) * c, c4, n, h, w, c, k, acc, j * c, c4)
            return acc[:, :c].to(buf.dtype), None
        L = _lib()
        st = L.stream_ptr()
        dd = _rows_dense(d)
        if dd.dtype == buf.dtype:
            out = ops.empty_nhwc(n, c, h, w, buf)
            rc = L.lib().ly_sppf_bwd(L.ptr(buf), c4, L.ptr(dd), c4, n, h, w, c, k, L.ptr(out), c, L.dtype_code(buf), st)
            if rc == 0:
                return out, None
            if rc != 1:
                L.check(rc, "ly_sppf_bwd")
        at = lambda t, off: ctypes.c_void_p(t.data_ptr() + t.element_size() * off)
        arg = torch.empty((n * h * w, 3 * c), dtype=torch.uint8, device=buf.device)
        L.check(L.lib().ly_maxpool_arg(L.ptr(buf), c4, n, h, w, 3 * c, k, L.ptr(arg), 3 * c, L.dtype_code(buf), st), "ly_maxpool_arg")
        up = dd[:, 3 * c:].float().contiguous(memory_format=torch.channels_last)
        tmp = [torch.empty((n * h * w, c), dtype=torch.float32, device=buf.device) for _ in range(2)]
        out = ops.empty_nhwc(n, c, h, w, buf)
        up_p, up_ld = ops.rows(up)
        for j in (2, 1, 0):
            dst = out if j == 0 else tmp[j & 1]
            L.check(L.lib().ly_maxpool_gather(at(arg, j * c), 3 * c, L.ptr(up_p) if j == 2 else L.ptr(tmp[(j + 1) & 1]), c, at(dd, j * c), c4, L.dtype_code(dd),
                                              n, h, w, c, k, L.ptr(dst), c, L.dtype_code(dst), st), "ly_maxpool_gather")
        return out, None


def _lib():
    from . import capi
    return capi


DEBUG_TAP = None


def _tap(name, t):
    if DEBUG_TAP is not None:
        DEBUG_TAP(name, t)


class RfcbamFn(torch.autograd.Function):
    @staticmethod
    def forward(ctx, mod, x, se_wa, se_wb, gen_w, gen_gamma, gen_beta, getw, conv_w, conv_b, out_gamma, out_beta):
        xr, ld = ops.rows(x)
        n, c, h, w = xr.shape
        k, s, o = mod.kernel_size, mod.stride, mod.o
        ho, wo = (h + 2 * (k // 2) - k) // s + 1, (w + 2 * (k // 2) - k) // s + 1
# ... 377 lines not shown
```

### lead-yolo_amd/modules.py

```python
import torch
import torch.nn as nn
import torch.nn.functional as F

from . import ops, pack
from .ops import ACT_NONE, ACT_RELU, ACT_SILU

BN_EPS = 1e-3
BN_MOMENTUM = 0.03


class _Prepared:

    def __init__(self):
        self.slots = {}

    def get(self, key, build, variant=0):
        ent = self.slots.get(variant)
        if ent is None or ent[0] != key or (torch.is_grad_enabled() and torch.cuda.is_current_stream_capturing()):
            with torch.no_grad():
                ent = (key, build())
            self.slots[variant] = ent
        return ent[1]

    def __deepcopy__(self, memo):
# ... 358 lines not shown

def autopad(k, p=None, d=1):
    if d > 1:
        k = d * (k - 1) + 1 if isinstance(k, int) else [d * (x - 1) + 1 for x in k]
    if p is None:
        p = k // 2 if isinstance(k, int) else [x // 2 for x in k]
    return p


class Conv(nn.Module):
    default_act = nn.SiLU()

    def __init__(self, c1, c2, k=1, s=1, p=None, g=1, d=1, act=True):
        super().__init__()
        if g != 1 or d != 1 or k not in (1, 3) or autopad(k, p, d) != k // 2 or s not in (1, 2) or (s == 2 and k != 3):
            raise NotImplementedError(f"HIP Conv is built for k in (1, 3), stride 1 (k = 3 also stride 2, inference), groups 1, 'same' padding "
                                      f"(got k={k} s={s} g={g} d={d}); grouped / depthwise Conv (DWConv) is not used by LEAD-YOLO and not built")
        self.s = s
        self.conv = nn.Conv2d(c1, c2, k, s, autopad(k, p, d), groups=g, dilation=d, bias=False)
        if k == 3:
            self.conv.weight._ly_tap_major = True
        self.bn = nn.BatchNorm2d(c2)
        self.act = self.default_act if act is True else act if isinstance(act, nn.Module) else nn.Identity()
        self.k, self.c1, self.c2 = k, c1, c2
        self._prep = _Prepared()
        self._prep_bn = _Prepared()

    def weights(self, planes=2):
        conv = self.conv
        key = pack.versions(conv.weight)

        def build():
            w = conv.weight
            if self.k == 1:
                return pack.packed(pack.src_matrix(w, self.c2, self.c1), self.c1, planes)
            cip = (self.c1 + 31) // 32 * 32
            return pack.packed(pack.src_taps(w, cip), 9 * cip, planes)
        return self._prep.get(key, build, planes)

    def affine_eval(self):
        conv, bn = self.conv, getattr(self, "bn", None)
        key = pack.versions(conv.bias, *(_bn_tensors(bn) if bn is not None else ())) + (bn.eps if bn is not None else 0,)

        def build():
            if bn is not None:
                return pack.bn_scale_shift(bn, conv.bias)
            return None, (conv.bias.detach().float().contiguous() if conv.bias is not None else None)
        return self._prep_bn.get(key, build)

    def _run(self, x, sc, sh, act, stats=None):
        wp = self.weights(ops.planes_of(x.a0 if isinstance(x, Lazy) else x))
        if self.k == 1:
            return _run_pointwise(x, wp, self.c2, sc, sh, act, stats=stats)
        xr, ld = ops.rows(x)
        n, c, h, w = xr.shape
        out = None if stats is not None else ops.empty_nhwc(n, self.c2, h, w, xr)
        ops.conv3x3(M=n * h * w, H=h, W=w, Cin=c, N=self.c2, x=xr, ldx=ld, wp=wp, out=out, ldo=self.c2, e_scale=sc, e_shift=sh, act=act,
                    stats=stats)
        return out

    @_edge
    def forward(self, x):
        s_ = getattr(self, "s", 1)
        pr = _probe(x, (x.shape[0], self.c2, (x.shape[2] - 1) // s_ + 1, (x.shape[3] - 1) // s_ + 1)) if isinstance(x, torch.Tensor) else None
        if pr is not None:
            return pr
        if self.k == 3 and isinstance(x, Lazy):
            x = x.materialize()
        act = _act_code(self.act)
        bn = getattr(self, "bn", None)
        if getattr(self, "s", 1) == 2:
            if self.training:
                raise NotImplementedError("HIP Conv with stride 2 is built for inference (eval mode) only")
            sc, sh = self.affine_eval()
            return self._run(x, sc, sh, act)[:, :, ::2, ::2].contiguous(memory_format=torch.channels_last)
        if _grad_mode(self) and bn is not None:
            from . import grad
            x0, x1, up = x, None, False
            if isinstance(x, Lazy):
                if x.gate is not None:
                    x0 = x.materialize()
                else:
                    x0, x1, up = x.keep[0], (x.keep[1] if x.a1 is not None else None), x.up
            spec = grad.ConvSpec("pw" if self.k == 1 else "c3", self.c2, act, bn, True, up=up)
            return grad.conv_bn_act(spec, self.weights(ops.planes_of(x0)), x0, x1, self.conv.weight, self.conv.bias, bn)
        if self.training and bn is not None:
            L = Lazy.of(x)
            n, _, h, w = L.shape
            bias = self.conv.bias.detach().float().contiguous() if self.conv.bias is not None else None
            stats = ops.new_stats(self.c2, L.a0.device)
            self._run(x, None, bias, ACT_NONE, stats=stats)
            sc, sh = ops.bn_finalize(bn, stats, self.c2, n * h * w, bias=bias)
        else:
            sc, sh = self.affine_eval()
        return self._run(x, sc, sh, act)

    def forward_fuse(self, x):
        return self.forward(x)


class SE(nn.Module):
    def __init__(self, in_channel, ratio=16):
        super().__init__()
        self.gap = nn.AdaptiveAvgPool2d((1, 1))
        self.fc = nn.Sequential(nn.Linear(in_channel, ratio, bias=False), nn.ReLU(), nn.Linear(ratio, in_channel, bias=False),
                                nn.Sigmoid())
        self.ratio = ratio

    def attention(self, xr, ld, n, hw, c):
        wa, wb = self.fc[0].weight.detach(), self.fc[2].weight.detach()
        return ops.se_attention(xr, ld, n, hw, c, wa.contiguous(), wb.contiguous(), self.ratio)

    def forward(self, x):
        x, _ = ops.edge_in(x, "SE", self)
        xr, ld = ops.rows(x)
        n, c, h, w = xr.shape
        return self.attention(xr, ld, n, h * w, c).view(n, c, 1, 1)


class RFCBAMConv(nn.Module):
    def __init__(self, in_channel, out_channel, kernel_size=3, stride=1, dilation=1):
        super().__init__()
        k = kernel_size
        if k not in (1, 3):
            raise NotImplementedError("HIP RFCBAMConv is built for kernel_size 1 and 3")
        if k == 1 and stride != 1:
            raise NotImplementedError("HIP RFCBAMConv with kernel_size 1 is built for stride 1")
        if k == 3 and in_channel % 16 != 0:
            raise NotImplementedError("HIP RFCBAMConv with kernel_size 3 needs in_channel % 16 == 0")
        self.kernel_size, self.stride = k, stride
        self.c, self.o = in_channel, out_channel
        self.generate = nn.Sequential(nn.Conv2d(in_channel, in_channel * k * k, k, padding=k // 2, stride=stride, groups=in_channel,
                                                bias=False), nn.BatchNorm2d(in_channel * k * k), nn.ReLU())
        self.get_weight = nn.Sequential(nn.Conv2d(2, 1, kernel_size=3, padding=1, bias=False), nn.Sigmoid())
        self.se = SE(in_channel)
        self.conv = nn.Sequential(nn.Conv2d(in_channel, out_channel, k, stride=k), nn.BatchNorm2d(out_channel), nn.ReLU())
        if k > 1:
            self.conv[0].weight._ly_tap_major = True
        self._prep = _Prepared()

    def _packed(self, planes=2):
        gw, gbn, cw, cbn = self.generate[0].weight, self.generate[1], self.conv[0], self.conv[1]
        key = pack.versions(gw, *_bn_tensors(gbn), cw.weight, cw.bias, *_bn_tensors(cbn), self.get_weight[0].weight) + (gbn.eps, cbn.eps, RF3M)

        def build():
            k, c, o = self.kernel_size, self.c, self.o
            gs, gb = pack.bn_scale_shift(gbn)
            w18 = self.get_weight[0].weight.detach().float().reshape(18).contiguous()
            es, eb = pack.bn_scale_shift(cbn, cw.bias)
            if k == 1:
                a1 = (gw.detach().float().view(c) * gs).contiguous()
                return dict(a1=a1, b1=gb, w18=w18, wp=pack.packed(pack.src_matrix(cw.weight, o, c), c, planes), es=es, eb=eb)
            wq_stats = pack.rfcbam_gen_weights(gw, gs, gb, 32, False)
            wq_main = pack.rfcbam_gen_weights(gw, gs, gb, 16, True)
            wsrc = pack.Src(cw.weight, o, srb=c * 9, nb=10, vb=9, nc=16, sa=144, sb=1, sc=9)
            d = dict(wq_stats=wq_stats, wq_main=wq_main, w18=w18, wp=pack.packed(wsrc, (c // 16) * 160, planes), es=es, eb=eb)
            if ops.rf3c_ok(c, self.stride):
                d["wq_c"] = pack.rfcbam_gen_weights_c(gw, gs, gb)
                d["wp_c"] = self._wp_c(planes)
            if planes == 1 and RF3M and ops.rf3m_ok(torch.bfloat16, c, o, self.stride):
                d["wm_stats"] = pack.rf3m_stream(gw, gs, gb, pool_stride=self.stride)
                d["wm"] = pack.rf3m_stream(gw, gs, gb, cw.weight, 4 if o % 128 == 0 else 2)
            return d
        return self._prep.get(key, build, planes)

    def _wp_c(self, planes):
        cw, c = self.conv[0], self.c
# ... 119 lines not shown
        super().__init__()
        self.relu = nn.ReLU6(inplace=inplace)


class h_swish(nn.Module):
    def __init__(self, inplace=True):
        super().__init__()
        self.sigmoid = h_sigmoid(inplace=inplace)


class CoordAtt(nn.Module):
    def __init__(self, inp, oup, reduction=32):
        super().__init__()
        if inp != oup:
            raise NotImplementedError("HIP CoordAtt gates its own input: inp must equal oup")
        self.pool_h = nn.AdaptiveAvgPool2d((None, 1))
        self.pool_w = nn.AdaptiveAvgPool2d((1, None))
        mip = max(8, inp // reduction)
        self.conv1 = nn.Conv2d(inp, mip, kernel_size=1, stride=1, padding=0)
        self.bn1 = nn.BatchNorm2d(mip)
        self.act = h_swish()
        self.conv_h = nn.Conv2d(mip, oup, kernel_size=1, stride=1, padding=0)
        self.conv_w = nn.Conv2d(mip, oup, kernel_size=1, stride=1, padding=0)
        self.mip, self.c = mip, inp
        self._prep = _Prepared()
        self._prep_bn = _Prepared()
        self.trainable_on_hip = mip in (8, 16) and inp <= 512

    def train(self, mode=True):
        if mode and not self.trainable_on_hip and any(p.requires_grad for p in self.parameters()):
            raise NotImplementedError(f"CoordAtt(c={self.c}, mip={self.mip}): the HIP training path is built for mip in (8, 16) and c <= 512; this width "
                                      "runs in eval mode only (freeze the module's parameters or pick a width with c // 32 in {<= 8, 16})")
        return super().train(mode)

    def _weights(self):
        key = pack.versions(self.conv1.weight, self.conv1.bias, self.conv_h.weight, self.conv_h.bias, self.conv_w.weight, self.conv_w.bias)

        def build():
            f = lambda p: p.detach().float().reshape(p.shape[0], -1).contiguous()
            return (f(self.conv1.weight), self.conv1.bias.detach().float().contiguous(), f(self.conv_h.weight),
                    self.conv_h.bias.detach().float().contiguous(), f(self.conv_w.weight), self.conv_w.bias.detach().float().contiguous())
        return self._prep.get(key, build)

    def _conv1_eval(self):
        key = pack.versions(self.conv1.weight, self.conv1.bias, *_bn_tensors(self.bn1)) + (self.bn1.eps,)

        def build():
            s, t = pack.bn_scale_shift(self.bn1, self.conv1.bias)
            return (self.conv1.weight.detach().float().view(self.mip, self.c) * s.view(-1, 1)).contiguous(), t
        return self._prep_bn.get(key, build)

    def attention(self, xr, ld, n, h, w, c):
        w1raw, b1raw, wh, bh, ww, bw = self._weights()
        pool = ops.pool_hw(xr, ld, n, h, w, c)
        if self.training:
            st = ops.coordatt_conv1_stats(pool, n * (h + w), c, self.mip, w1raw, b1raw).float()
            sc, sh = ops.bn_batch_affine(self.bn1, st[:self.mip], st[self.mip:], n * (h + w))
            w1, b1 = (w1raw * sc.view(-1, 1)).contiguous(), (b1raw * sc + sh).contiguous()
        else:
            w1, b1 = self._conv1_eval()
        return ops.coordatt_mlp(pool, n, h, w, c, self.mip, w1, b1, wh, bh, ww, bw)

    @_edge
    def forward(self, x):
        pr = _probe(x, x.shape)
        if pr is not None:
            return pr
        if _grad_mode(self):
            from . import grad
            return grad.coordatt_train(self, x)
        xr, ld = ops.rows(x)
        n, c, h, w = xr.shape
        a_h, a_w = self.attention(xr, ld, n, h, w, c)
        return ops.coordatt_gate(xr, ld, n, h, w, c, a_h, a_w)


class CA_Bottleneck(nn.Module):
    def __init__(self, c1, c2, shortcut=True, g=1, e=0.5):
        super().__init__()
        c_ = int(c2 * e)
        self.cv1 = Conv(c1, c_, 1, 1)
        self.cv2 = Conv(c_, c2, 3, 1, g=g)
        self.ca = CoordAtt(c2, c2, 32)
        self.add = shortcut and c1 == c2

    def forward_lazy(self, x):
        if _grad_mode(self):
            xin = x.materialize() if isinstance(x, Lazy) else x
            y = self.ca(self.cv2(self.cv1(xin)))
            return xin + y if self.add else y
        src = Lazy.of(x)
        t1 = self.cv1(src)
        t2 = self.cv2(t1)
        n, c, h, w = t2.shape
        a_h, a_w = self.ca.attention(t2, c, n, h, w, c)
        if self.add:
            if src.gate is not None or src.a1 is not None or src.up:
                rr, ldr = ops.rows(src.materialize())
            else:
                rr, ldr = src.a0, src.lda0
            return ops.coordatt_gate(t2, c, n, h, w, c, a_h, a_w, rr, ldr)
        return Lazy((n, c, h, w), t2, c, c, gate=(a_h, a_w), keep=(t2, a_h, a_w))

    @_edge
    def forward(self, x):
        pr = _probe(x, (x.shape[0], self.cv2.c2, x.shape[2], x.shape[3])) if isinstance(x, torch.Tensor) else None
        if pr is not None:
            return pr
        y = self.forward_lazy(x)
        return y.materialize() if isinstance(y, Lazy) else y


class C3_CA(nn.Module):
    def __init__(self, c1, c2, n=1, shortcut=True, g=1, e=0.5):
        super().__init__()
        c_ = int(c2 * e)
        self.cv1 = Conv(c1, c_, 1, 1)
        self.cv2 = Conv(c1, c_, 1, 1)
        self.cv3 = Conv(2 * c_, c2, 1)
        self.m = nn.Sequential(*(CA_Bottleneck(c_, c_, shortcut, g, e=1.0) for _ in range(n)))
        self.c_, self.c2 = c_, c2
        self._prep = _Prepared()
        self._prep_bn = _Prepared()
        self.cv1.conv.weight._ly_grad_pair = self.cv2.conv.weight

    def _weights12(self, planes=2):
        p1, p2 = self.cv1, self.cv2
        key = pack.versions(p1.conv.weight, p2.conv.weight)
        c1 = p1.conv.weight.shape[1]

        def build():
            if self.c_ % 16 == 0:
                return pack.packed([pack.src_matrix(p1.conv.weight, self.c_, c1), pack.src_matrix(p2.conv.weight, self.c_, c1)], c1, planes)
            return pack.frag_pack3(torch.cat((p1.conv.weight.detach().view(self.c_, -1), p2.conv.weight.detach().view(self.c_, -1)), 0), planes=planes)
        return self._prep.get(key, build, planes)

    def _cv12_train(self, x):
        p1, p2 = self.cv1, self.cv2
        b1, b2 = getattr(p1, "bn", None), getattr(p2, "bn", None)
        gated = isinstance(x, Lazy) and x.gate is not None
        if (b1 is None or b2 is None or not (b1.training and b2.training) or p1.k != 1 or p2.k != 1 or p1.conv.bias is not None
                or p2.conv.bias is not None or gated or self.c_ % 16 or b1.weight is None or b2.weight is None):
            return self.cv1(x), self.cv2(x)
        from . import grad
        if pack.src_matrix_kcat_t(p1.conv.weight, p2.conv.weight) is None:
            return self.cv1(x), self.cv2(x)
        x0, x1, up = x, None, False
        if isinstance(x, Lazy):
            x0, x1, up = x.keep[0], (x.keep[1] if x.a1 is not None else None), x.up
        return grad.conv_bn_act_pair(_act_code(p1.act), up, self._weights12(ops.planes_of(x0)), x0, x1, p1.conv, b1, p2.conv, b2)

    def _affine12_eval(self):
        p1, p2 = self.cv1, self.cv2
        b1, b2 = getattr(p1, "bn", None), getattr(p2, "bn", None)
        key = pack.versions(p1.conv.bias, p2.conv.bias, *(_bn_tensors(b1) if b1 is not None else ()),
                            *(_bn_tensors(b2) if b2 is not None else ()))

        def build():
            parts = []
            for p, b in ((p1, b1), (p2, b2)):
                if b is not None:
                    parts.append(pack.bn_scale_shift(b, p.conv.bias))
                else:
                    parts.append((torch.ones(self.c_, device=p.conv.weight.device), p.conv.bias.detach().float()))
            return torch.cat((parts[0][0], parts[1][0])).contiguous(), torch.cat((parts[0][1], parts[1][1])).contiguous()
        return self._prep_bn.get(key, build)
# ... 263 lines not shown
```

### lead-yolo_amd/ops.py

```python
import ctypes
import os

import torch

from . import capi
from .capi import (ACT_NONE, ACT_RELU, ACT_SILU, GATHER_PATCH, GATHER_PATCH_NCHW, GATHER_PATCH_NCHW_BF16, GATHER_PATCH_NCHW_F16, GATHER_PATCH_NCHW_U8, GATHER_ROWS, GATHER_UP2,
                   PRO_AFFINE_RELU_CA, PRO_GATE, PRO_NONE)


PROFILE = None


class _Timed:

    def __init__(self, name, flops, nbytes, valu_flops=0.0):
        self.rec = None
        if PROFILE is not None:
            self.rec = [name, float(flops), float(nbytes), torch.cuda.Event(enable_timing=True), torch.cuda.Event(enable_timing=True), float(valu_flops)]

    def __enter__(self):
        if self.rec is not None:
            self.rec[3].record()

    def __exit__(self, *a):
# ... 111 lines not shown
    x = nhwc(x)
    if x.stride(1) != 1:
        x = x.permute(0, 2, 3, 1).contiguous().permute(0, 3, 1, 2)
    return x, c


_p = capi.ptr


def gemm(*, M, H, W, K, N, a0, lda0, k0, wp, out, ldo, a1=None, lda1=0, gather=GATHER_ROWS, Hin=0, Win=0, Cin=0, ks=0, pk=0,
         pro=PRO_NONE, g_h=None, g_w=None, res=None, ldres=0, p_scale=None, p_shift=None, p_ca=None, e_scale=None,
         e_shift=None, rowscale=None, act=ACT_NONE, stats=None, dtype=None, scat_ks=0, scat_c=0, eadd=None, ldeadd=0):
    if gather == GATHER_PATCH_NCHW:
        gather = {torch.uint8: GATHER_PATCH_NCHW_U8, torch.bfloat16: GATHER_PATCH_NCHW_BF16, torch.float16: GATHER_PATCH_NCHW_F16}.get(a0.dtype, gather)
    image = gather in (GATHER_PATCH_NCHW, GATHER_PATCH_NCHW_U8, GATHER_PATCH_NCHW_BF16, GATHER_PATCH_NCHW_F16)
    dt = (out if out is not None else a0).dtype if not image or out is not None else torch.float32
    if dtype is not None:
        dt = dtype
    code = capi.dtype_code(dt)
    P = capi.LyGemmParams(M, H, W, K, N, _p(a0), lda0, k0, _p(a1), lda1, gather, Hin, Win, Cin, ks, pk, pro, _p(g_h), _p(g_w),
                          _p(res), ldres, _p(p_scale), _p(p_shift), _p(p_ca), _p(wp), _p(e_scale), _p(e_shift), _p(rowscale),
                          act, _p(out), ldo, _p(stats), code, scat_ks, scat_c, _p(eadd), ldeadd)
    if eadd is not None and eadd.dtype != out.dtype:
        raise ValueError("gemm: eadd must have the output's dtype")
    nt, mt, wc = gemm_config(N)
    ti = {GATHER_PATCH_NCHW_U8: "unsigned char", GATHER_PATCH_NCHW_BF16: "ly_bf16img", GATHER_PATCH_NCHW_F16: "ly_f16img"}.get(
        gather, "float" if (code == 0 or image) else "__bf16")
    to = "float" if code == 0 else "__bf16"
    es_i, es_o = {"float": 4, "__bf16": 2, "unsigned char": 1, "ly_bf16img": 2, "ly_f16img": 2}[ti], (4 if to == "float" else 2)
    kgather = GATHER_PATCH_NCHW if image else gather
    nchunk = -(-K // (128 if ti == "__bf16" else 64))
    nch = 0
    if N % 4 == 0 and ldo % 4 == 0 and out is not None:
        ok1 = wc == 4 or pro == 0
        ok2 = wc == 4 and pro != PRO_GATE
        if stats is not None:
            ok1, ok2 = ok1 and pro != PRO_GATE, ok2 and pro == 0
        nch = 1 if (nchunk == 1 and ok1) else 2 if (nchunk == 2 and ok2) else 0
    fast = N % 4 == 0 and ldo % 4 == 0 and out is not None
    ep = (2 if stats is not None else 1) if (nch or (fast and pro == 0)) else 1 if (fast and pro == PRO_GATE and stats is None) else 0
    if scat_ks or eadd is not None:
        ep = 4 if eadd is not None else 3
    name = f"ly_gemm_kernel_d2<{ti}, {to}, {nt}, {mt}, {wc}, {kgather}, {pro}, {nch}, {ep}>"
    if (image and Cin == 3 and K == 48 and 20 <= N <= 80 and N % 4 == 0 and (out is None or ldo % 4 == 0) and Hin == 4 * H and Win == 4 * W
            and (code != 0 or gather in (GATHER_PATCH_NCHW, GATHER_PATCH_NCHW_U8))):
        name = f"ly_patch4_kernel<{ti}, {to}, {max(2, -(-N // 16))}, {'true' if stats is not None else 'false'}>"
    with _Timed(name, 2.0 * M * K * N, es_i * M * K + (es_o * M * N if out is not None else 0) + 4.0 * N * K):
        capi.check(capi.lib().ly_gemm_fwd(ctypes.byref(P), capi.stream_ptr()), "ly_gemm_fwd")


def mlpblock_pconv(x, z, n, h, w, c, wp):
    with _Timed(f"ly_mlpblock_persist_kernel<{_tname(x)}, {c}, pconv>", 18.0 * n * h * w * (c // 4) ** 2, 2.0 * x.element_size() * n * h * w * c):
        rc = capi.lib().ly_mlpblock_pconv(_p(x), _p(z), n, h, w, c, _p(wp), capi.dtype_code(x), capi.stream_ptr())
    if rc < 0:
        capi.check(rc, "ly_mlpblock_pconv")
    return rc == 0


def conv3x3(*, M, H, W, Cin, N, x, ldx, wp, out, ldo, e_scale=None, e_shift=None, act=ACT_NONE, stats=None):
    th, tw = pick_conv_tile(H, W)
    code = capi.dtype_code(x)
    P = capi.LyConv3Params(M, H, W, Cin, N, th, tw, _p(x), ldx, _p(wp), _p(e_scale), _p(e_shift), act, _p(out), ldo, _p(stats), code)
    mt, wc = (2, 4) if N > 64 else (2, 2)
    ntv = -(-(th * tw) // 16)
    nta = 0 if code == 0 else (ntv if (wc == 4 and ntv in (5, 8)) else 4 if (wc == 2 and ntv == 8) else 0)
    name = f"ly_conv3x3_kernel<{_tname(x)}, {mt}, {wc}, {nta}>"
    if code != 0 and N > 64 and (M // (H * W)) * -(-W // tw) * -(-H // th) * -(-N // 128) < 512:
        name = "ly_conv3x3_lat_kernel<__bf16, 2, 2>"
    with _Timed(name, 2.0 * M * 9 * Cin * N, x.element_size() * M * (Cin + N) + 4.0 * 9 * Cin * N):
        capi.check(capi.lib().ly_conv3x3_fwd(ctypes.byref(P), capi.stream_ptr()), "ly_conv3x3_fwd")


def _tname(t):
    return "float" if t.dtype == torch.float32 else "__bf16"


def pool_hw(x, ldx, n, h, w, c):
    pool = torch.empty((n, h + w, c), dtype=torch.float32, device=x.device)
    with _Timed(f"ly_pool_hw_kernel<{_tname(x)}>", 1.0 * n * h * w * c, x.element_size() * n * h * w * c):
        capi.check(capi.lib().ly_pool_hw(_p(x), ldx, n, h, w, c, _p(pool), capi.dtype_code(x), capi.stream_ptr()), "ly_pool_hw")
    return pool


def coordatt_mlp(pool, n, h, w, c, mip, w1, b1, wh, bh, ww, bw, sc=None, sh=None):
    a_h = torch.empty((n, h, c), dtype=torch.float32, device=pool.device)
    a_w = torch.empty((n, w, c), dtype=torch.float32, device=pool.device)
    capi.check(capi.lib().ly_coordatt_mlp(_p(pool), n, h, w, c, mip, _p(w1), _p(b1), _p(sc), _p(sh), _p(wh), _p(bh), _p(ww), _p(bw), _p(a_h),
                                          _p(a_w), capi.stream_ptr()), "ly_coordatt_mlp")
    return a_h, a_w


def coordatt_mlp_bwd(pool, n, h, w, c, mip, w1, b1, mean, invstd, gamma, beta, wh, ww, a_h, a_w, da_h, da_w, targets):
    r = n * (h + w)
    sums = zeros_f64(32 * 2 * mip, pool.device)
    ws = torch.empty(r * 3 * mip, dtype=torch.float32, device=pool.device)
    dpool = torch.empty((n, h + w, c), dtype=torch.float32, device=pool.device)
    with _Timed("ly_coordatt_mlp_bwd1_kernel + bwd2", 8.0 * r * c * mip, 4.0 * 4 * r * c):
        capi.check(capi.lib().ly_coordatt_mlp_bwd(_p(pool), n, h, w, c, mip, _p(w1), _p(b1), _p(mean), _p(invstd), _p(gamma), _p(beta), _p(wh), _p(ww),
                                                  _p(a_h), _p(a_w), _p(da_h), _p(da_w), _p(ws), _p(sums), _p(dpool),
                                                  *[_p(t) for t in targets], int(targets[0].dtype == torch.float64), capi.stream_ptr()),
                   "ly_coordatt_mlp_bwd")
    return dpool


def coordatt_gate(x, ldx, n, h, w, c, a_h, a_w, res=None, ldres=0):
    out = empty_nhwc(n, c, h, w, x)
    with _Timed(f"ly_gate_kernel<{_tname(x)}>", 2.0 * n * h * w * c, 2.0 * x.element_size() * n * h * w * c):
        capi.check(capi.lib().ly_coordatt_gate(_p(x), ldx, n, h, w, c, _p(a_h), _p(a_w), _p(res), ldres, _p(out), c, capi.dtype_code(x),
                                               capi.stream_ptr()), "ly_coordatt_gate")
    return out


def se_attention(x, ldx, n, hw, c, wa, wb, r, want_part=False):
    slices = se_slices(hw)
    part = torch.empty((n, slices, c), dtype=torch.float32, device=x.device)
    ca = torch.empty((n, c), dtype=torch.float32, device=x.device)
    with _Timed(f"ly_colsum_kernel<{_tname(x)}> + ly_se_mlp_kernel", 1.0 * n * hw * c, x.element_size() * n * hw * c):
        capi.check(capi.lib().ly_se_fwd(_p(x), ldx, n, hw, c, _p(wa), _p(wb), r, _p(part), slices, _p(ca), capi.dtype_code(x), capi.stream_ptr()),
                   "ly_se_fwd")
    return (ca, part) if want_part else ca


def se_bwd(part, n, hw, c, wa, wb, r, ca, d_ca, dwa, dwb):
    if d_ca.dtype not in (torch.float32, torch.float64) or d_ca.numel() != n * c or not d_ca.is_contiguous():
        raise ValueError("se_bwd: d_ca must be a contiguous float32 / float64 [n, c]")
    dgap = torch.empty((n, c), dtype=torch.float32, device=part.device)
    ws = torch.empty(n * (2 * c + 2 * r), dtype=torch.float32, device=part.device)
    capi.check(capi.lib().ly_se_bwd(_p(part), part.shape[1], n, hw, c, _p(wa), _p(wb), r, _p(ca), _p(d_ca), int(d_ca.dtype == torch.float64), _p(dwa), _p(dwb), _p(dgap), _p(ws),
                                    capi.stream_ptr()), "ly_se_bwd")
    return dgap


def se_slices(hw):
    return max(1, min(hw // 64, 128))


def colsum(x, ldx, n, hw, c):
    slices = se_slices(hw)
    part = torch.empty((n, slices, c), dtype=torch.float32, device=x.device)
    with _Timed(f"ly_colsum_kernel<{_tname(x)}>", 1.0 * n * hw * c, x.element_size() * n * hw * c):
        capi.check(capi.lib().ly_colsum(_p(x), ldx, n, hw, c, _p(part), slices, capi.dtype_code(x), capi.stream_ptr()), "ly_colsum")
    return part


def pick_tile(ho, wo):
    best = None
    for nct in range(1, 9):
        tw = -(-wo // nct)
        if tw > 64:
            continue
        th = max(1, 64 // tw)
        th = min(th, ho)
        nrt = -(-ho // th)
        eff = (ho * wo) / (nct * nrt * 64.0)
        if best is None or eff > best[0] + 1e-9:
            best = (eff, th, tw)
    if best is None:
        return 1, 64
    return best[1], best[2]


def rf3c_ok(c, s):
    return c % 32 == 0 and s in (1, 2)


RF3M_MIN_UNITS = 1500
# ... 583 lines not shown


def bn_batch_affine(bn, s1, s2, count):
    return bn_batch_stats(bn, s1, s2, count)[:2]


_TRIU = None


def rfcbam_generate_stats(x, ldx, n, h, w, c, s, gen_w):
    global _TRIU
    mom = torch.zeros(54, c, dtype=torch.float64, device=x.device)
    with _Timed(f"ly_rfcbam_tap_moments_kernel<{_tname(x)}>", 108.0 * n * h * w * c / (s * s), x.element_size() * n * h * w * c):
        capi.check(capi.lib().ly_rfcbam_tap_moments(_p(x), ldx, n, h, w, c, s, _p(mom), capi.dtype_code(x), capi.stream_ptr()), "ly_rfcbam_tap_moments")
    mom = mom.float()
    if _TRIU is None or _TRIU[0].device != x.device:
        iu = torch.triu_indices(9, 9, device=x.device)
        _TRIU = (iu[0], iu[1])
    m1 = mom[:9].t()
    M = torch.zeros(c, 9, 9, dtype=torch.float32, device=x.device)
    M[:, _TRIU[0], _TRIU[1]] = mom[9:].t()
    M = M + M.transpose(1, 2) - torch.diag_embed(torch.diagonal(M, dim1=1, dim2=2))
    wv = gen_w.detach().float().view(c, 9, 9)
    s1 = torch.einsum("ctu,cu->ct", wv, m1)
    s2 = torch.einsum("ctu,cuv,ctv->ct", wv, M, wv)
    ho, wo = (h + 2 - 3) // s + 1, (w + 2 - 3) // s + 1
    return s1.reshape(-1), s2.reshape(-1), n * ho * wo


def rfcbam_gen_prepare(x, ldx, n, h, w, c, k, s, gen_w, bn):
    kk = k * k
    dev = x.device
    if k == 3:
        mom = zeros_f64(54 * c, dev)
        with _Timed(f"ly_rfcbam_tap_moments_kernel<{_tname(x)}>", 108.0 * n * h * w * c / (s * s), x.element_size() * n * h * w * c):
            capi.check(capi.lib().ly_rfcbam_tap_moments(_p(x), ldx, n, h, w, c, s, _p(mom), capi.dtype_code(x), capi.stream_ptr()), "ly_rfcbam_tap_moments")
        ho, wo = (h + 2 - 3) // s + 1, (w + 2 - 3) // s + 1
        count = n * ho * wo
    else:
        mom = chan_moments(x, ldx, n * h * w, c, striped=True)
        count = n * h * w
    g = c * kk
    out8 = torch.empty(8, g, dtype=torch.float32, device=dev)
    a1 = torch.empty(c, dtype=torch.float32, device=dev) if k == 1 else None
    cps, cpm = (c + 31) // 32 * 32, (c + 15) // 16 * 16
    wqs = torch.empty(cps * 90, dtype=torch.float32, device=dev) if k == 3 else None
    wqm = torch.empty(cpm * 90, dtype=torch.float32, device=dev) if k == 3 else None
    wqc = torch.empty(c * 100, dtype=torch.float32, device=dev) if (k == 3 and c % 32 == 0) else None
    if bn.weight.dtype != torch.float32:
        raise NotImplementedError("train-mode BatchNorm needs float32 parameters and buffers")
    track = bn.track_running_stats and bn.running_mean is not None
    capi.check(capi.lib().ly_rfcbam_gen_prepare(_p(mom), c, k, _p(gen_w.detach()), _p(bn.weight.detach()), _p(bn.bias.detach()), float(bn.eps),
                                                float(bn.momentum or 0.0), float(count), _p(bn.running_mean if track else None),
                                                _p(bn.running_var if track else None), _p(bn.num_batches_tracked if track else None), _p(out8),
                                                _p(a1), _p(wqs), _p(wqm), _p(wqc), mom.shape[0] if k == 1 else 1, capi.stream_ptr()), "ly_rfcbam_gen_prepare")
    from . import pack
    pack.touch()
    return dict(gs=out8[0], gb=out8[1], gmean=out8[2], ginv=out8[3], ag=out8[4], bg=out8[5], gmean_tc=out8[6], ginv_tc=out8[7], a1=a1,
                wq_stats=wqs, wq_main=wqm, wq_c=wqc)


def bn_batch_stats(bn, s1, s2, count):
    with torch.no_grad():
        mean = s1 / count
        var = (s2 / count - mean * mean).clamp_(min=0.0)
        invstd = torch.rsqrt(var + bn.eps)
        scale = bn.weight.detach().float() * invstd
        shift = bn.bias.detach().float() - mean * scale
        if bn.track_running_stats and bn.running_mean is not None:
            mom = bn.momentum if bn.momentum is not None else 1.0 / float(bn.num_batches_tracked + 1)
            bn.running_mean.mul_(1.0 - mom).add_(mean, alpha=mom)
            bn.running_var.mul_(1.0 - mom).add_(var * (count / max(count - 1, 1)), alpha=mom)
            bn.num_batches_tracked += 1
    return scale.contiguous(), shift.contiguous(), mean, invstd


def bnact_fwd(u, ldu, rows, c, a, b, act, y, ldy):
    with _Timed(f"ly_bnact_fwd_kernel<{_tname(u)}, {act}>", 4.0 * rows * c, 2.0 * u.element_size() * rows * c):
        capi.check(capi.lib().ly_bnact_fwd(_p(u), ldu, rows, c, _p(a), _p(b), act, _p(y), ldy, capi.dtype_code(u), capi.stream_ptr()), "ly_bnact_fwd")


def bnact_bwd_reduce(dy, lddy, u, ldu, rows, c, a, b, act):
    sums = new_stats(c, u.device)
    with _Timed(f"ly_bnact_bwd_reduce_kernel<{_tname(u)}, {act}>", 6.0 * rows * c, 2.0 * u.element_size() * rows * c):
        capi.check(capi.lib().ly_bnact_bwd_reduce(_p(dy), lddy, _p(u), ldu, rows, c, _p(a), _p(b), act, _p(sums), capi.dtype_code(u),
                                                  capi.stream_ptr()), "ly_bnact_bwd_reduce")
    return sums


def bnact_bwd_apply(dy, lddy, u, ldu, rows, c, a, b, act, alpha, kappa, lam, du, lddu):
    with _Timed(f"ly_bnact_bwd_apply_kernel<{_tname(u)}, {act}>", 8.0 * rows * c, 3.0 * u.element_size() * rows * c):
        capi.check(capi.lib().ly_bnact_bwd_apply(_p(dy), lddy, _p(u), ldu, rows, c, _p(a), _p(b), act, _p(alpha), _p(kappa), _p(lam),
                                                 _p(du), lddu, capi.dtype_code(u), capi.stream_ptr()), "ly_bnact_bwd_apply")


def bnact_bwd_reduce_pair(dy1, lddy1, dy2, lddy2, csplit, u, ldu, rows, c, a, b, act):
    s1, s2 = new_stats(csplit, u.device), new_stats(c - csplit, u.device)
    with _Timed(f"ly_bnact_bwd_reduce_kernel<{_tname(u)}, {act}>", 6.0 * rows * c, 2.0 * u.element_size() * rows * c):
        capi.check(capi.lib().ly_bnact_bwd_reduce_pair(_p(dy1), lddy1, _p(dy2), lddy2, csplit, _p(u), ldu, rows, c, _p(a), _p(b), act, _p(s1), _p(s2),
                                                       capi.dtype_code(u), capi.stream_ptr()), "ly_bnact_bwd_reduce_pair")
    return s1, s2


def bnact_bwd_apply_pair(dy1, lddy1, dy2, lddy2, csplit, u, ldu, rows, c, a, b, act, alpha, kappa, lam, du, lddu):
    with _Timed(f"ly_bnact_bwd_apply_kernel<{_tname(u)}, {act}>", 8.0 * rows * c, 3.0 * u.element_size() * rows * c):
        capi.check(capi.lib().ly_bnact_bwd_apply_pair(_p(dy1), lddy1, _p(dy2), lddy2, csplit, _p(u), ldu, rows, c, _p(a), _p(b), act, _p(alpha), _p(kappa),
                                                      _p(lam), _p(du), lddu, capi.dtype_code(u), capi.stream_ptr()), "ly_bnact_bwd_apply_pair")


def wgrad(*, M, H, W, N, du, lddu, x, ldx, Hin, Win, Cin, dw, lddw, ks=1, stride=1, pad=0, nchw=False, up2=False, du_off=0, x_off=0,
          dw_off=0, dw_ts=None, dw_cs=1, n_valid=None, c_valid=None, x_scale=None, x_shift=None, _now=False):
    q = dict(M=M, H=H, W=W, N=N, du=du, lddu=lddu, x=x, ldx=ldx, Hin=Hin, Win=Win, Cin=Cin, dw=dw, lddw=lddw, ks=ks, stride=stride,
             pad=pad, nchw=nchw, up2=up2, du_off=du_off, x_off=x_off, dw_off=dw_off, dw_ts=dw_ts, dw_cs=dw_cs, n_valid=n_valid,
             c_valid=c_valid, x_scale=x_scale, x_shift=x_shift)
    if not _now and _wgrad_deferrable(q):
        return _wgrad_enqueue(q)
    P = _wgrad_params(**q)
    with _Timed(wgrad_kernel_name(_tname(x), N, ks * ks * Cin, ks == 1 and stride == 1 and pad == 0 and not nchw and not up2,
                                  (not nchw) and N % 4 == 0 and Cin % 4 == 0 and lddu % 4 == 0 and ldx % 4 == 0, x_scale is not None,
                                  _wgrad_octets(x, du, N, Cin, lddu, ldx, du_off, x_off)),
                2.0 * M * N * ks * ks * Cin, x.element_size() * M * (N + Cin) + 4.0 * N * ks * ks * Cin):
        capi.check(capi.lib().ly_wgrad(ctypes.byref(P), capi.stream_ptr()), "ly_wgrad")


def _wgrad_params(*, M, H, W, N, du, lddu, x, ldx, Hin, Win, Cin, dw, lddw, ks=1, stride=1, pad=0, nchw=False, up2=False, du_off=0, x_off=0,
                  dw_off=0, dw_ts=None, dw_cs=1, n_valid=None, c_valid=None, x_scale=None, x_shift=None):
    def at(t, off):
        return ctypes.c_void_p(t.data_ptr() + t.element_size() * off)
    if du.dtype != x.dtype:
        raise capi.HipLibraryError(f"wgrad: du ({du.dtype}) and x ({x.dtype}) must share one storage dtype")
    if (x_scale is None) != (x_shift is None):
        raise ValueError("wgrad: x_scale and x_shift come together")
    if x_scale is not None and (x_scale.dtype != torch.float32 or x_shift.dtype != torch.float32 or x_scale.numel() < Cin or x_shift.numel() < Cin):
        raise ValueError("wgrad: x_scale / x_shift must be float32 vectors of at least Cin elements")
    ws = wgrad_workspace(x.device)
    return capi.LyWgradParams(M, H, W, N, at(du, du_off), lddu, at(x, x_off), ldx, Hin, Win, Cin, ks, stride, pad, int(nchw), int(up2),
                              at(dw, dw_off), lddw, capi.dtype_code(x), Cin if dw_ts is None else dw_ts, dw_cs, N if n_valid is None else n_valid,
                              Cin if c_valid is None else c_valid, _p(x_scale), _p(x_shift), _p(ws), ws.numel() if ws is not None else 0)


WGRAD_WS_FLOATS = 24 << 20
_WGRAD_WS = {}


def wgrad_workspace(device):
    if WGRAD_WS_FLOATS <= 0:
        return None
    ws = _WGRAD_WS.get(device)
    if ws is None:
        if torch.cuda.is_current_stream_capturing():
            return None
        ws = _WGRAD_WS[device] = torch.empty(WGRAD_WS_FLOATS, dtype=torch.float32, device=device)
    return ws


def _wgrad_groupable(q, dtype):
    return (q.get("ks", 1) == 1 and q.get("stride", 1) == 1 and q.get("pad", 0) == 0 and not q.get("nchw") and not q.get("up2")
            and q["N"] > 64 and q["N"] % 4 == 0 and q["Cin"] % 4 == 0 and q["lddu"] % 4 == 0 and q["ldx"] % 4 == 0
            and q["Hin"] == q["H"] and q["Win"] == q["W"] and q["x"].dtype == dtype)


class _WgradQueue:
    items = []
    notify = []
    task = -1


WGRAD_DEFER = True
WGRAD_GROUP_MAX = 4
WGRAD_DEFER_MAX_MACS = 4 << 30


def _wgrad_deferrable(q):
    return (WGRAD_DEFER and SINK is not None and q["x"].dtype == torch.bfloat16 and _wgrad_groupable(q, torch.bfloat16)
            and q["Cin"] > 64 and q["M"] * q["N"] * q["Cin"] <= WGRAD_DEFER_MAX_MACS and q.get("dw_off", 0) == 0 and SINK.is_target(q["dw"]) and _graph_task() >= 0)


def _wgrad_span(q):
    lo = q["dw"].data_ptr() + 4 * q.get("dw_off", 0)
    return lo, lo + 4 * q["N"] * q["lddw"]


def _wgrad_enqueue(q):
    task = _graph_task()
    if _WgradQueue.task != task:
        _WgradQueue.items, _WgradQueue.notify, _WgradQueue.task = [], [], task
        torch.autograd.Variable._execution_engine.queue_callback(wgrad_flush)
    lo, hi = _wgrad_span(q)
# ... 153 lines not shown
```

Baseline: 7012 images/sec.

## Fuse CoordAtt pooling into preceding conv BN-act forward and backward kernels

Adds a fused BN+activation kernel that also computes the CoordAtt H/W average pools while writing the activation, so the separate pool_hw pass over the feature map is skipped. In backward, the pool gradient is folded into the BN-act reduce/apply kernels by gathering per-row/column pooled gradients on the fly, which removes the separate pool_hw_bwd scatter pass. A cross-module link object carries the pool and dpool between the Conv and CoordAtt autograd functions. The cost is extra gather loads and index arithmetic in the hot backward kernels, a lower unroll factor in the apply kernel, and more fragile coupling between modules.

Result: no change. 7019 images/sec (median of 6 runs) (+0.1%).

```diff
diff --git a/include/lead_yolo_hip.h b/include/lead_yolo_hip.h
--- a/include/lead_yolo_hip.h
+++ b/include/lead_yolo_hip.h
@@ -223,6 +223,13 @@
 int ly_bnact_bwd_apply_pair(const void* dy1 , int lddy1, const void* dy2 , int lddy2, int csplit, const void* u , int ldu, long rows, int C,
                             const float* a, const float* b, int act, const float* alpha, const float* kappa, const float* lambda, void* du , int lddu,
                             int dtype, void* stream);
+int ly_bnact_bwd_reduce_pool(const void* dy , int lddy, const void* u , int ldu, int n_img, int H, int W, int C, const float* a, const float* b,
+                             int act, const float* gp , double* sums, int dtype, void* stream);
+int ly_bnact_bwd_apply_pool(const void* dy , int lddy, const void* u , int ldu, int n_img, int H, int W, int C, const float* a, const float* b,
+                            int act, const float* gp, const float* alpha, const float* kappa, const float* lambda, void* du , int lddu, int dtype,
+                            void* stream);
+int ly_bnact_pool_fwd(const void* u , int ldu, int n_img, int H, int W, int C, const float* a, const float* b, int act, void* y , int ldy,
+                      float* pool, int dtype, void* stream);
 
 typedef struct LyWgradParams {
   long M;
diff --git a/lead-yolo_amd/csrc/ly_attention.hip b/lead-yolo_amd/csrc/ly_attention.hip
--- a/lead-yolo_amd/csrc/ly_attention.hip
+++ b/lead-yolo_amd/csrc/ly_attention.hip
@@ -38,6 +38,64 @@
   LY_CHECK(x && pool && (C & 3) == 0 && (ldx & 3) == 0 && C <= 1024, "pool_hw: bad arguments (C=%d ldx=%d)", C, ldx);
   LY_WITH_T(dtype, hipLaunchKernelGGL(ly_pool_hw_kernel<T>, dim3(n_img * (H + W)), dim3(LY_THREADS), 0, reinterpret_cast<hipStream_t>(stream),
                                       reinterpret_cast<const T*>(x), ldx, H, W, C, pool));
+  LY_LAUNCH_CHECK();
+  return 0;
+}
+
+template <typename T, int ACT>
+__global__ __launch_bounds__(LY_THREADS) void ly_bnact_pool_fwd_kernel(const T* __restrict__ u, int ldu, int H, int W, int C, const float* __restrict__ a,
+                                                                        const float* __restrict__ b, T* __restrict__ y, int ldy, float* __restrict__ pool) {
+  __shared__ f32x4 red[LY_THREADS];
+  const int L = H + W;
+  const int bid = ly_xcd_remap((int)blockIdx.x, (int)gridDim.x);
+  const int n = bid / L, pos = bid - n * L;
+  const int nc4 = C >> 2;
+  const int tid = threadIdx.x;
+  const int groups = LY_THREADS / nc4;
+  const bool row = pos < H;
+  const int len = row ? W : H;
+  const long base = row ? ((long)n * H + pos) * W : ((long)n * H) * W + (pos - H);
+  const long step = row ? 1 : W;
+  const int c4 = tid % nc4, j0 = tid / nc4;
+  f32x4 s = ly_zero4();
+  if (j0 < groups) {
+    const f32x4 av = ly_ldg4(a + 4 * c4), bv = ly_ldg4(b + 4 * c4);
+    if (row) {
+#pragma unroll 4
+      for (int j = j0; j < len; j += groups) {
+        const f32x4 v = ly_act4(av * ly_ld4<T>(u + (base + j) * ldu + 4 * c4) + bv, ACT);
+        ly_st4<T>(y + (base + j) * ldy + 4 * c4, v);
+        s += ly_round4<T>(v);
+      }
+    } else {
+#pragma unroll 4
+      for (int j = j0; j < len; j += groups) s += ly_round4<T>(ly_act4(av * ly_ld4<T>(u + (base + j * step) * ldu + 4 * c4) + bv, ACT));
+    }
+  }
+  red[tid] = s;
+  __syncthreads();
+  if (j0 == 0) {
+    for (int g = 1; g < groups; ++g) s += red[g * nc4 + c4];
+    const float inv = 1.f / (float)len;
+    ly_stg4(pool + ((long)n * L + pos) * C + 4 * c4, s * inv);
+  }
+}
+
+extern "C" int ly_bnact_pool_fwd(const void* u_, int ldu, int n_img, int H, int W, int C, const float* a, const float* b, int act, void* y_, int ldy,
+                                 float* pool, int dtype, void* stream) {
+  LY_CHECK_DTYPE(dtype, "bnact_pool_fwd");
+  LY_CHECK(u_ && a && b && y_ && pool && n_img > 0 && H > 0 && W > 0, "bnact_pool_fwd: bad arguments");
+  LY_CHECK((C & 3) == 0 && C > 0 && C <= 1024 && (ldu & 3) == 0 && (ldy & 3) == 0, "bnact_pool_fwd: bad arguments (C=%d ldu=%d ldy=%d)", C, ldu, ldy);
+  LY_CHECK((long)n_img * (H + W) < (1L << 31), "bnact_pool_fwd: too many rows");
+  hipStream_t st = reinterpret_cast<hipStream_t>(stream);
+  const dim3 grid((unsigned)(n_img * (H + W)));
+  LY_WITH_T(dtype, {
+    const T* u = reinterpret_cast<const T*>(u_);
+    T* y = reinterpret_cast<T*>(y_);
+    if (act == LY_ACT_SILU) hipLaunchKernelGGL((ly_bnact_pool_fwd_kernel<T, LY_ACT_SILU>), grid, dim3(LY_THREADS), 0, st, u, ldu, H, W, C, a, b, y, ldy, pool);
+    else if (act == LY_ACT_RELU) hipLaunchKernelGGL((ly_bnact_pool_fwd_kernel<T, LY_ACT_RELU>), grid, dim3(LY_THREADS), 0, st, u, ldu, H, W, C, a, b, y, ldy, pool);
+    else hipLaunchKernelGGL((ly_bnact_pool_fwd_kernel<T, LY_ACT_NONE>), grid, dim3(LY_THREADS), 0, st, u, ldu, H, W, C, a, b, y, ldy, pool);
+  });
   LY_LAUNCH_CHECK();
   return 0;
 }
diff --git a/lead-yolo_amd/csrc/ly_backward.hip b/lead-yolo_amd/csrc/ly_backward.hip
--- a/lead-yolo_amd/csrc/ly_backward.hip
+++ b/lead-yolo_amd/csrc/ly_backward.hip
@@ -43,11 +43,63 @@
   const long xw_begin = xw_lo + (xw_on ? xw_slot : (long)blockIdx.x) * (groups_);                                         \
   const long xw_step = (xw_on ? xw_n : (long)gridDim.x) * (groups_)
 
-template <typename T, int ACT>
+struct LyPoolAdd {
+  const float* gp;
+  int H, W, vec;
+  float iw, ih;
+};
+__device__ __forceinline__ f32x4 ly_pool_grad_vec(f32x4 ghw , const f32x4 gw, const float ih, const f32x4 o) {
+  f32x4 v;
+#pragma unroll
+  for (int i = 0; i < 4; ++i) {
+    float t = ghw[i];
+    asm("" : "+v"(t));
+    v[i] = __builtin_fmaf(gw[i], ih, t);
+    asm("" : "+v"(v[i]));
+  }
+  v += o;
+  return v;
+}
+__device__ __forceinline__ f32x4 ly_pool_grad_flat(const f32x4 gh, const f32x4 gw, const float iw, const float ih, const f32x4 o) {
+  f32x4 v;
+#pragma unroll
+  for (int i = 0; i < 4; ++i) {
+    float t = gw[i] * ih;
+    asm("" : "+v"(t));
+    v[i] = __builtin_fmaf(gh[i], iw, t);
+    asm("" : "+v"(v[i]));
+  }
+  v += o;
+  return v;
+}
+__device__ __forceinline__ f32x4 ly_pool_grad(const LyPoolAdd& A, const f32x4 gh, const f32x4 gw, const f32x4 o) {
+  return A.vec ? ly_pool_grad_vec(gh * A.iw, gw, A.ih, o) : ly_pool_grad_flat(gh, gw, A.iw, A.ih, o);
+}
+struct LyRowPos { int n, h, w; };
+__device__ __forceinline__ LyRowPos ly_rowpos(const long r, const int H, const int W) {
+  const unsigned ur = (unsigned)r, row = ur / (unsigned)W;
+  LyRowPos p;
+  p.w = (int)(ur - row * (unsigned)W);
+  p.n = (int)(row / (unsigned)H);
+  p.h = (int)(row - (unsigned)p.n * (unsigned)H);
+  return p;
+}
+__device__ __forceinline__ LyRowPos ly_rowpos_add(LyRowPos p, const LyRowPos d, const int H, const int W) {
+  p.w += d.w;
+  int cy = p.w >= W;
+  p.w -= cy ? W : 0;
+  p.h += d.h + cy;
+  cy = p.h >= H;
+  p.h -= cy ? H : 0;
+  p.n += d.n + cy;
+  return p;
+}
+
+template <typename T, int ACT, bool ADD>
 __global__ __launch_bounds__(LY_THREADS) void ly_bnact_bwd_reduce_kernel(const T* __restrict__ dy, int lddy, const T* __restrict__ u,
                                                                           int ldu, long rows, int C, const float* __restrict__ a,
                                                                           const float* __restrict__ b, double* __restrict__ sums,
-                                                                          const T* __restrict__ dy2, int lddy2, int csplit, double* __restrict__ sums2) {
+                                                                          const T* __restrict__ dy2, int lddy2, int csplit, double* __restrict__ sums2, const LyPoolAdd A) {
   __shared__ f32x4 red1[LY_THREADS], red2[LY_THREADS];
   using R4 = typename LyT<T>::R4;
   const int ncv = C >> 2, tid = threadIdx.x;
@@ -62,18 +114,40 @@
     const long stride = xw_step;
     const T* const dyb = second ? dy2 + (4 * cv - csplit) : dy + 4 * cv;
     const long ldd = second ? lddy2 : lddy;
+    LyRowPos pos[UR], dpos;
+    const float* gph = nullptr;
+    const float* gpw = nullptr;
+    int gimg = 0;
+    if constexpr (ADD) {
+      const long first = xw_begin + j0 < rows ? xw_begin + j0 : 0;
+#pragma unroll
+      for (int k = 0; k < UR; ++k) pos[k] = ly_rowpos(first + k * stride < rows ? first + k * stride : 0, A.H, A.W);
+      dpos = ly_rowpos(UR * stride, A.H, A.W);
+      gph = A.gp + 4 * cv;
+      gpw = gph + (long)A.H * C;
+      gimg = (A.H + A.W) * C;
+    }
     for (long r0 = xw_begin + j0; r0 < xw_end; r0 += UR * stride) {
       R4 qu[UR], qg[UR];
+      f32x4 gh[UR], gw[UR];
 #pragma unroll
       for (int k = 0; k < UR; ++k) {
-        const long r = r0 + k * stride < xw_end ? r0 + k * stride : xw_end - 1;
+        const bool ok = r0 + k * stride < xw_end;
+        const long r = ok ? r0 + k * stride : xw_end - 1;
         qu[k] = ly_ldr4<T>(u + r * ldu + 4 * cv);
         qg[k] = ly_ldr4<T>(dyb + r * ldd);
+        if constexpr (ADD) {
+          gh[k] = ly_ldg4(gph + (ok ? pos[k].n * gimg + pos[k].h * C : 0));
+          gw[k] = ly_ldg4(gpw + (ok ? pos[k].n * gimg + pos[k].w * C : 0));
+          pos[k] = ly_rowpos_add(pos[k], dpos, A.H, A.W);
+        }
       }
 #pragma unroll
       for (int k = 0; k < UR; ++k) {
         const f32x4 uu = ly_r4_f32(qu[k]);
-        f32x4 dv = ly_dact4<ACT>(av * uu + bv, ly_r4_f32(qg[k]));
+        f32x4 g = ly_r4_f32(qg[k]);
+        if constexpr (ADD) g = ly_round4<T>(ly_pool_grad(A, gh[k], gw[k], g));
+        f32x4 dv = ly_dact4<ACT>(av * uu + bv, g);
         if (!(r0 + k * stride < xw_end)) dv = ly_zero4();
         s1 += dv;
         s2 += dv * uu;
@@ -95,12 +169,12 @@
   }
 }
 
-template <typename T, int ACT>
+template <typename T, int ACT, bool ADD>
 __global__ __launch_bounds__(LY_THREADS) void ly_bnact_bwd_apply_kernel(const T* __restrict__ dy, int lddy, const T* u, int ldu,
                                                                          long rows, int C, const float* __restrict__ a,
                                                                          const float* __restrict__ b, const float* __restrict__ alpha,
                                                                          const float* __restrict__ kappa, const float* __restrict__ lambda,
-                                                                         T* du, int lddu, const T* __restrict__ dy2, int lddy2, int csplit) {
+                                                                         T* du, int lddu, const T* __restrict__ dy2, int lddy2, int csplit, const LyPoolAdd A) {
   constexpr int VW = LyT<T>::VW, NQ = VW / 4;
   using RV = typename LyT<T>::RV;
   if ((C % VW) == 0 && (ldu % VW) == 0 && (lddy % VW) == 0 && (lddu % VW) == 0 && (lddy2 % VW) == 0 && (csplit % VW) == 0 && C / VW <= LY_THREADS) {
@@ -117,19 +191,46 @@
     LY_XCD_ROWS(rows, groups);
     const T* const gb = c >= csplit ? dy2 + (c - csplit) : dy + c;
     const long ldg = c >= csplit ? lddy2 : lddy;
-    for (long r0 = xw_begin + j0; r0 < xw_end; r0 += LY_EW_UR * xw_step) {
-      RV qu[LY_EW_UR], qg[LY_EW_UR];
-#pragma unroll
-      for (int k = 0; k < LY_EW_UR; ++k) {
-        const long r = r0 + k * xw_step < xw_end ? r0 + k * xw_step : xw_end - 1;
+    constexpr int UR = ADD ? 2 : LY_EW_UR;
+    LyRowPos pos[UR], dpos;
+    const float* gph = nullptr;
+    const float* gpw = nullptr;
+    int gimg = 0;
+    if constexpr (ADD) {
+      const long first = xw_begin + j0 < rows ? xw_begin + j0 : 0;
+#pragma unroll
+      for (int k = 0; k < UR; ++k) pos[k] = ly_rowpos(first + k * xw_step < rows ? first + k * xw_step : 0, A.H, A.W);
+      dpos = ly_rowpos(UR * xw_step, A.H, A.W);
+      gph = A.gp + c;
+      gpw = gph + (long)A.H * C;
+      gimg = (A.H + A.W) * C;
+    }
+    for (long r0 = xw_begin + j0; r0 < xw_end; r0 += UR * xw_step) {
+      RV qu[UR], qg[UR];
+      f32x4 gh[UR][NQ], gw[UR][NQ];
+#pragma unroll
+      for (int k = 0; k < UR; ++k) {
+        const bool ok = r0 + k * xw_step < xw_end;
+        const long r = ok ? r0 + k * xw_step : xw_end - 1;
         qu[k] = ly_ldrv<T>(u + r * ldu + c);
         qg[k] = ly_ldrv<T>(gb + r * ldg);
-      }
-#pragma unroll
-      for (int k = 0; k < LY_EW_UR; ++k) {
+        if constexpr (ADD) {
+          const int oh = ok ? pos[k].n * gimg + pos[k].h * C : 0, ow = ok ? pos[k].n * gimg + pos[k].w * C : 0;
+#pragma unroll
+          for (int q = 0; q < NQ; ++q) { gh[k][q] = ly_ldg4(gph + oh + 4 * q); gw[k][q] = ly_ldg4(gpw + ow + 4 * q); }
+          pos[k] = ly_rowpos_add(pos[k], dpos, A.H, A.W);
+        }
+      }
+#pragma unroll
+      for (int k = 0; k < UR; ++k) {
         f32x4 uu[NQ], g[NQ];
         ly_rv_unpack(qu[k], uu);
         ly_rv_unpack(qg[k], g);
+        if constexpr (ADD) {
+#pragma unroll
+          for (int q = 0; q < NQ; ++q) g[q] = ly_pool_grad(A, gh[k][q], gw[k][q], g[q]);
+          ly_rv_unpack(ly_rv_pack(g, (RV*)nullptr), g);
+        }
 #pragma unroll
         for (int q = 0; q < NQ; ++q) {
           const f32x4 dv = ly_dact4<ACT>(ca[q] * uu[q] + cb[q], g[q]);
@@ -148,7 +249,12 @@
     const long r = i / nc4;
     const int c = 4 * (int)(i - r * nc4);
     const f32x4 uu = ly_ld4<T>(u + r * ldu + c);
-    const f32x4 g = ly_ld4<T>(c >= csplit ? dy2 + r * lddy2 + (c - csplit) : dy + r * lddy + c);
+    f32x4 g = ly_ld4<T>(c >= csplit ? dy2 + r * lddy2 + (c - csplit) : dy + r * lddy + c);
+    if constexpr (ADD) {
+      const LyRowPos p = ly_rowpos(r, A.H, A.W);
+      const float* const gn = A.gp + (long)p.n * (A.H + A.W) * C + c;
+      g = ly_round4<T>(ly_pool_grad(A, ly_ldg4(gn + (long)p.h * C), ly_ldg4(gn + (long)(A.H + p.w) * C), g));
+    }
     const f32x4 dv = ly_dact4<ACT>(ly_ldg4(a + c) * uu + ly_ldg4(b + c), g);
     ly_st4<T>(du + r * lddu + c, ly_ldg4(alpha + c) * dv + ly_ldg4(kappa + c) + ly_ldg4(lambda + c) * uu);
   }
@@ -231,8 +337,15 @@
   return 0;
 }
 
+static const LyPoolAdd LY_NO_POOL_ADD = {nullptr, 0, 0, 0, 0.f, 0.f};
+static LyPoolAdd ly_pool_add(const float* gp, int H, int W, int C, int lddy, int dtype) {
+  const int vw = dtype == LY_BF16 ? 8 : 4;
+  LyPoolAdd A = {gp, H, W, (C % vw) == 0 && (lddy % vw) == 0 && C / vw <= LY_THREADS, 1.f / (float)W, 1.f / (float)H};
+  return A;
+}
+
 static int bnact_bwd_reduce_launch(const void* dy_, int lddy, const void* dy2_, int lddy2, int csplit, const void* u_, int ldu, long rows, int C, const float* a,
-                                   const float* b, int act, double* sums, double* sums2, int dtype, void* stream) {
+                                   const float* b, int act, double* sums, double* sums2, int dtype, void* stream, const LyPoolAdd A = LY_NO_POOL_ADD) {
   const int vw = 4;
   const int groups = LY_THREADS / (C / vw);
 #ifndef LY_RED_ROWS
@@ -242,7 +355,11 @@
   blocks = blocks < 1 ? 1 : blocks > 2048 ? 2048 : blocks;
   if (blocks >= 8) blocks = (blocks + 7) / 8 * 8;
   hipStream_t st = reinterpret_cast<hipStream_t>(stream);
-#define LY_RED(A) hipLaunchKernelGGL((ly_bnact_bwd_reduce_kernel<T, A>), dim3((unsigned)blocks), dim3(LY_THREADS), 0, st, dy, lddy, u, ldu, rows, C, a, b, sums, dy2, lddy2, csplit, sums2)
+#define LY_RED(ACT_)                                                                                                                                 \
+  do {                                                                                                                                               \
+    if (A.gp) hipLaunchKernelGGL((ly_bnact_bwd_reduce_kernel<T, ACT_, true>), dim3((unsigned)blocks), dim3(LY_THREADS), 0, st, dy, lddy, u, ldu, rows, C, a, b, sums, dy2, lddy2, csplit, sums2, A); \
+    else hipLaunchKernelGGL((ly_bnact_bwd_reduce_kernel<T, ACT_, false>), dim3((unsigned)blocks), dim3(LY_THREADS), 0, st, dy, lddy, u, ldu, rows, C, a, b, sums, dy2, lddy2, csplit, sums2, A); \
+  } while (0)
   LY_WITH_T(dtype, {
     const T* dy = reinterpret_cast<const T*>(dy_);
     const T* dy2 = reinterpret_cast<const T*>(dy2_);
@@ -274,12 +391,17 @@
 }
 
 static int bnact_bwd_apply_launch(const void* dy_, int lddy, const void* dy2_, int lddy2, int csplit, const void* u_, int ldu, long rows, int C, const float* a,
-                                  const float* b, int act, const float* alpha, const float* kappa, const float* lambda, void* du_, int lddu, int dtype, void* stream) {
+                                  const float* b, int act, const float* alpha, const float* kappa, const float* lambda, void* du_, int lddu, int dtype, void* stream,
+                                  const LyPoolAdd A = LY_NO_POOL_ADD) {
   const int vw_ = dtype == LY_BF16 ? 8 : 4;
   const bool vec_ = (C % vw_) == 0 && (ldu % vw_) == 0 && (lddy % vw_) == 0 && (lddu % vw_) == 0 && (lddy2 % vw_) == 0 && (csplit % vw_) == 0 && C / vw_ <= LY_THREADS;
   const long blocks = vec_ ? ly_ew_row_blocks(rows, C, vw_) : ly_ew_blocks(rows * (C >> 2));
   hipStream_t st = reinterpret_cast<hipStream_t>(stream);
-#define LY_APP(A) hipLaunchKernelGGL((ly_bnact_bwd_apply_kernel<T, A>), dim3((unsigned)blocks), dim3(LY_THREADS), 0, st, dy, lddy, u, ldu, rows, C, a, b, alpha, kappa, lambda, du, lddu, dy2, lddy2, csplit)
+#define LY_APP(ACT_)                                                                                                                                 \
+  do {                                                                                                                                               \
+    if (A.gp) hipLaunchKernelGGL((ly_bnact_bwd_apply_kernel<T, ACT_, true>), dim3((unsigned)blocks), dim3(LY_THREADS), 0, st, dy, lddy, u, ldu, rows, C, a, b, alpha, kappa, lambda, du, lddu, dy2, lddy2, csplit, A); \
+    else hipLaunchKernelGGL((ly_bnact_bwd_apply_kernel<T, ACT_, false>), dim3((unsigned)blocks), dim3(LY_THREADS), 0, st, dy, lddy, u, ldu, rows, C, a, b, alpha, kappa, lambda, du, lddu, dy2, lddy2, csplit, A); \
+  } while (0)
   LY_WITH_T(dtype, {
     const T* dy = reinterpret_cast<const T*>(dy_);
     const T* dy2 = reinterpret_cast<const T*>(dy2_);
@@ -311,6 +433,30 @@
            "bnact_bwd_apply_pair: C=%d csplit=%d / ld must be multiples of 4", C, csplit);
   return bnact_bwd_apply_launch(dy1, lddy1, dy2, lddy2, csplit, u_, ldu, rows, C, a, b, act, alpha, kappa, lambda, du_, lddu, dtype, stream);
 }
+
+#define LY_CHECK_POOL_ADD(who)                                                                                                                \
+  LY_CHECK(gp && n_img > 0 && H > 0 && W > 0, who ": bad map shape");                                                                          \
+  LY_CHECK((long)n_img * H * W < (1L << 31) && (long)n_img * (H + W) * C < (1L << 31), who ": map too large for 32-bit row arithmetic")
+extern "C" int ly_bnact_bwd_reduce_pool(const void* dy_, int lddy, const void* u_, int ldu, int n_img, int H, int W, int C, const float* a, const float* b,
+                                        int act, const float* gp, double* sums, int dtype, void* stream) {
+  LY_CHECK_DTYPE(dtype, "bnact_bwd_reduce_pool");
+  LY_CHECK(dy_ && u_ && a && b && sums, "bnact_bwd_reduce_pool: null pointer");
+  LY_CHECK((C & 3) == 0 && C > 0 && C <= 1024 && (lddy & 3) == 0 && (ldu & 3) == 0, "bnact_bwd_reduce_pool: C=%d / ld must be multiples of 4", C);
+  LY_CHECK_POOL_ADD("bnact_bwd_reduce_pool");
+  return bnact_bwd_reduce_launch(dy_, lddy, dy_, lddy, C, u_, ldu, (long)n_img * H * W, C, a, b, act, sums, sums, dtype, stream,
+                                 ly_pool_add(gp, H, W, C, lddy, dtype));
+}
+extern "C" int ly_bnact_bwd_apply_pool(const void* dy_, int lddy, const void* u_, int ldu, int n_img, int H, int W, int C, const float* a, const float* b,
+                                       int act, const float* gp, const float* alpha, const float* kappa, const float* lambda, void* du_, int lddu,
+                                       int dtype, void* stream) {
+  LY_CHECK_DTYPE(dtype, "bnact_bwd_apply_pool");
+  LY_CHECK(dy_ && u_ && a && b && alpha && kappa && lambda && du_, "bnact_bwd_apply_pool: null pointer");
+  LY_CHECK((C & 3) == 0 && C > 0 && (lddy & 3) == 0 && (ldu & 3) == 0 && (lddu & 3) == 0, "bnact_bwd_apply_pool: C=%d / ld must be multiples of 4", C);
+  LY_CHECK_POOL_ADD("bnact_bwd_apply_pool");
+  return bnact_bwd_apply_launch(dy_, lddy, dy_, lddy, C, u_, ldu, (long)n_img * H * W, C, a, b, act, alpha, kappa, lambda, du_, lddu, dtype, stream,
+                                ly_pool_add(gp, H, W, C, lddy, dtype));
+}
+#undef LY_CHECK_POOL_ADD
 
 __device__ __forceinline__ void ly_split8(const float (&v)[8], bf16x8& hi, bf16x8& lo) {
   bf16x4 h0, l0, h1, l1;
diff --git a/lead-yolo_amd/csrc/ly_tile.hpp b/lead-yolo_amd/csrc/ly_tile.hpp
--- a/lead-yolo_amd/csrc/ly_tile.hpp
+++ b/lead-yolo_amd/csrc/ly_tile.hpp
@@ -61,6 +61,10 @@
 template <typename T> __device__ __forceinline__ void ly_st4(T* p, const f32x4 v);
 template <> __device__ __forceinline__ void ly_st4<float>(float* p, const f32x4 v) { *reinterpret_cast<f32x4*>(p) = v; }
 template <> __device__ __forceinline__ void ly_st4<__bf16>(__bf16* p, const f32x4 v) { *reinterpret_cast<bf16x4*>(p) = ly_cvtb4(v); }
+template <typename T> __device__ __forceinline__ f32x4 ly_round4(const f32x4 v) {
+  if constexpr (LyT<T>::BF) return ly_cvt4(ly_cvtb4(v));
+  else return v;
+}
 template <typename T> __device__ __forceinline__ float ly_ld1(const T* p) { return (float)*p; }
 template <typename T> __device__ __forceinline__ void ly_st1(T* p, float v) { *p = (T)v; }
 
diff --git a/lead-yolo_amd/grad.py b/lead-yolo_amd/grad.py
--- a/lead-yolo_amd/grad.py
+++ b/lead-yolo_amd/grad.py
@@ -73,13 +73,21 @@
     return None
 
 
+class _CaLink:
+    __slots__ = ("pool", "dpool", "dx")
+
+    def __init__(self):
+        self.pool = self.dpool = self.dx = None
+
+
 class ConvSpec:
 
-    def __init__(self, kind, cout, act=ACT_NONE, bn=None, bn_train=False, k=1, nchw=False, up=False, out_dtype=None):
+    def __init__(self, kind, cout, act=ACT_NONE, bn=None, bn_train=False, k=1, nchw=False, up=False, out_dtype=None, pool_out=False):
         self.kind = kind
         self.cout, self.act, self.bn, self.bn_train = cout, act, bn, bn_train
         self.k, self.nchw, self.up = k, nchw, up
         self.out_dtype = out_dtype
+        self.pool_out = pool_out
 
 
 
@@ -127,11 +135,14 @@
 
 
 
-def affine_backward(dy, u, a, b, act, mean, invstd, train, inplace=True, gamma=None, beta=None, lddy=None, out=None):
+def affine_backward(dy, u, a, b, act, mean, invstd, train, inplace=True, gamma=None, beta=None, lddy=None, out=None, pool_add=None):
     n, c, h, w = u.shape
     rows = n * h * w
     lddy = c if lddy is None else lddy
-    sums = ops.bnact_bwd_reduce(dy, lddy, u, c, rows, c, a, b, act)
+    if pool_add is not None:
+        sums = ops.bnact_bwd_reduce_pool(dy, lddy, u, c, n, h, w, c, a, b, act, pool_add)
+    else:
+        sums = ops.bnact_bwd_reduce(dy, lddy, u, c, rows, c, a, b, act)
     tg, tb = ops.grad_target(gamma), ops.grad_target(beta)
     direct = tg is not None and tb is not None and tg.numel() == c and tb.numel() == c
     dgamma, dbeta, alpha, kappa, lam = ops.bn_bwd_coeffs(sums, c, rows, a, mean, invstd, train, dgamma=tg if direct else None,
@@ -140,7 +151,10 @@
         ops.grad_done(gamma)
         ops.grad_done(beta)
     du = out if out is not None else u if inplace else torch.empty_like(u)
-    ops.bnact_bwd_apply(dy, lddy, u, c, rows, c, a, b, act, alpha, kappa, lam, du, c)
+    if pool_add is not None:
+        ops.bnact_bwd_apply_pool(dy, lddy, u, c, n, h, w, c, a, b, act, pool_add, alpha, kappa, lam, du, c)
+    else:
+        ops.bnact_bwd_apply(dy, lddy, u, c, rows, c, a, b, act, alpha, kappa, lam, du, c)
     return du, dgamma, dbeta
 
 
@@ -279,7 +293,12 @@
                 rows = u.shape[0] * u.shape[2] * u.shape[3]
                 a, b, mean, invstd = ops.bn_finalize(spec.bn, stats, co, rows, want_stats=True)
                 y = torch.empty_like(u)
-                ops.bnact_fwd(u, co, rows, co, a, b, spec.act, y, co)
+                ctx.calink = None
+                if spec.pool_out and co <= 1024:
+                    ctx.calink = y._ly_calink = _CaLink()
+                    ctx.calink.pool = ops.bnact_pool_fwd(u, co, u.shape[0], u.shape[2], u.shape[3], co, a, b, spec.act, y, co)
+                else:
+                    ops.bnact_fwd(u, co, rows, co, a, b, spec.act, y, co)
                 ctx.spec, ctx.wp = spec, wp
                 ctx.has = (x1 is not None, bias is not None)
                 ctx.params = (weight, gamma, beta)
@@ -325,13 +344,19 @@
             dgamma = dbeta = dbias = None
             if spec.bn is not None or spec.act != ACT_NONE:
                 u = u_saved if u_saved is not None else _conv_forward(spec, x0, x1, wp, None, bias_f, ACT_NONE)
+                link, dpool = getattr(ctx, "calink", None), None
+                if link is not None and link.dpool is not None:
+                    dpool, dx_ca, link.dpool, link.dx = link.dpool, link.dx, None, None
+                    if not (dy.data_ptr() == dx_ca.data_ptr() and dy.shape == u.shape and dy.dtype == u.dtype and lddy == co):
+                        dy = ops.pool_hw_bwd(dpool, u.shape[0], u.shape[2], u.shape[3], co, into=_rows_dense(dy).clone())
+                        lddy, dpool = co, None
                 if spec.bn is None:
                     a = torch.ones(co, dtype=torch.float32, device=dy.device)
                     b = torch.zeros_like(a)
                     mean, invstd = b, a
                 du, dgamma, dbeta = affine_backward(dy, u, a, b, spec.act, mean, invstd, spec.bn is not None and spec.bn_train,
                                                     inplace=u_saved is None, gamma=g_param if spec.bn is not None else None,
-                                                    beta=b_param if spec.bn is not None else None, lddy=lddy)
+                                                    beta=b_param if spec.bn is not None else None, lddy=lddy, pool_add=dpool)
                 if bias_f is not None:
                     if spec.bn is None:
                         dbias, dgamma, dbeta = dbeta, None, None
@@ -721,7 +746,14 @@
         n, c, h, w = t.shape
         mip = mod.mip
         W1, Wh, Ww = (p.detach().reshape(p.shape[0], -1) for p in (w1, wh, ww))
-        pool = ops.pool_hw(t, ld, n, h, w, c)
+        link = getattr(x, "_ly_calink", None)
+        if link is not None and not (link.pool is not None and t.data_ptr() == x.data_ptr() and ld == c and tuple(link.pool.shape) == (n, h + w, c)):
+            link = None
+        if link is not None:
+            pool, link.pool = link.pool, None
+        else:
+            pool = ops.pool_hw(t, ld, n, h, w, c)
+        ctx.calink = link
         st = ops.coordatt_conv1_stats(pool, n * (h + w), c, mip, W1, b1)
         sc, sh, mean, invstd = ops.bn_finalize(mod.bn1, st.view(1, -1), mip, n * (h + w), want_stats=True)
         a_h, a_w = ops.coordatt_mlp(pool, n, h, w, c, mip, W1, b1.detach(), Wh, bh.detach(), Ww, bw.detach(), sc=sc, sh=sh)
@@ -771,7 +803,10 @@
                 out.append(rounded[k] if r is not None else None)
                 k += 1
             ret = out
-        ops.pool_hw_bwd(dpool, n, h, w, c, into=dx)
+        if ctx.calink is not None and ctx.needs_input_grad[1]:
+            ctx.calink.dpool, ctx.calink.dx = dpool, dx
+        else:
+            ops.pool_hw_bwd(dpool, n, h, w, c, into=dx)
         for i, (p, r) in enumerate(zip(ctx.params, ret)):
             if r is None and p.requires_grad and not (defer and i != 1):
                 ops.grad_done(p)
diff --git a/lead-yolo_amd/modules.py b/lead-yolo_amd/modules.py
--- a/lead-yolo_amd/modules.py
+++ b/lead-yolo_amd/modules.py
@@ -464,7 +464,7 @@
                     x0 = x.materialize()
                 else:
                     x0, x1, up = x.keep[0], (x.keep[1] if x.a1 is not None else None), x.up
-            spec = grad.ConvSpec("pw" if self.k == 1 else "c3", self.c2, act, bn, True, up=up)
+            spec = grad.ConvSpec("pw" if self.k == 1 else "c3", self.c2, act, bn, True, up=up, pool_out=getattr(self, "feeds_coordatt", False))
             return grad.conv_bn_act(spec, self.weights(ops.planes_of(x0)), x0, x1, self.conv.weight, self.conv.bias, bn)
         if self.training and bn is not None:
             L = Lazy.of(x)
@@ -750,6 +750,7 @@
         self.cv1 = Conv(c1, c_, 1, 1)
         self.cv2 = Conv(c_, c2, 3, 1, g=g)
         self.ca = CoordAtt(c2, c2, 32)
+        self.cv2.feeds_coordatt = True
         self.add = shortcut and c1 == c2
 
     def forward_lazy(self, x):
diff --git a/lead-yolo_amd/ops.py b/lead-yolo_amd/ops.py
--- a/lead-yolo_amd/ops.py
+++ b/lead-yolo_amd/ops.py
@@ -217,6 +217,14 @@
     return pool
 
 
+def bnact_pool_fwd(u, ldu, n, h, w, c, a, b, act, y, ldy):
+    pool = torch.empty((n, h + w, c), dtype=torch.float32, device=u.device)
+    with _Timed(f"ly_bnact_pool_fwd_kernel<{_tname(u)}, {act}>", 5.0 * n * h * w * c, 2.0 * u.element_size() * n * h * w * c):
+        capi.check(capi.lib().ly_bnact_pool_fwd(_p(u), ldu, n, h, w, c, _p(a), _p(b), act, _p(y), ldy, _p(pool), capi.dtype_code(u),
+                                                capi.stream_ptr()), "ly_bnact_pool_fwd")
+    return pool
+
+
 def coordatt_mlp(pool, n, h, w, c, mip, w1, b1, wh, bh, ww, bw, sc=None, sh=None):
     a_h = torch.empty((n, h, c), dtype=torch.float32, device=pool.device)
     a_w = torch.empty((n, w, c), dtype=torch.float32, device=pool.device)
@@ -966,28 +974,44 @@
 
 def bnact_bwd_reduce(dy, lddy, u, ldu, rows, c, a, b, act):
     sums = new_stats(c, u.device)
-    with _Timed(f"ly_bnact_bwd_reduce_kernel<{_tname(u)}, {act}>", 6.0 * rows * c, 2.0 * u.element_size() * rows * c):
+    with _Timed(f"ly_bnact_bwd_reduce_kernel<{_tname(u)}, {act}, false>", 6.0 * rows * c, 2.0 * u.element_size() * rows * c):
         capi.check(capi.lib().ly_bnact_bwd_reduce(_p(dy), lddy, _p(u), ldu, rows, c, _p(a), _p(b), act, _p(sums), capi.dtype_code(u),
                                                   capi.stream_ptr()), "ly_bnact_bwd_reduce")
     return sums
 
 
 def bnact_bwd_apply(dy, lddy, u, ldu, rows, c, a, b, act, alpha, kappa, lam, du, lddu):
-    with _Timed(f"ly_bnact_bwd_apply_kernel<{_tname(u)}, {act}>", 8.0 * rows * c, 3.0 * u.element_size() * rows * c):
+    with _Timed(f"ly_bnact_bwd_apply_kernel<{_tname(u)}, {act}, false>", 8.0 * rows * c, 3.0 * u.element_size() * rows * c):
         capi.check(capi.lib().ly_bnact_bwd_apply(_p(dy), lddy, _p(u), ldu, rows, c, _p(a), _p(b), act, _p(alpha), _p(kappa), _p(lam),
                                                  _p(du), lddu, capi.dtype_code(u), capi.stream_ptr()), "ly_bnact_bwd_apply")
 
 
+def bnact_bwd_reduce_pool(dy, lddy, u, ldu, n, h, w, c, a, b, act, gp):
+    sums = new_stats(c, u.device)
+    rows = n * h * w
+    with _Timed(f"ly_bnact_bwd_reduce_kernel<{_tname(u)}, {act}, true>", 6.0 * rows * c, 2.0 * u.element_size() * rows * c):
+        capi.check(capi.lib().ly_bnact_bwd_reduce_pool(_p(dy), lddy, _p(u), ldu, n, h, w, c, _p(a), _p(b), act, _p(gp), _p(sums), capi.dtype_code(u),
+                                                       capi.stream_ptr()), "ly_bnact_bwd_reduce_pool")
+    return sums
+
+
+def bnact_bwd_apply_pool(dy, lddy, u, ldu, n, h, w, c, a, b, act, gp, alpha, kappa, lam, du, lddu):
+    rows = n * h * w
+    with _Timed(f"ly_bnact_bwd_apply_kernel<{_tname(u)}, {act}, true>", 8.0 * rows * c, 3.0 * u.element_size() * rows * c):
+        capi.check(capi.lib().ly_bnact_bwd_apply_pool(_p(dy), lddy, _p(u), ldu, n, h, w, c, _p(a), _p(b), act, _p(gp), _p(alpha), _p(kappa), _p(lam),
+                                                      _p(du), lddu, capi.dtype_code(u), capi.stream_ptr()), "ly_bnact_bwd_apply_pool")
+
+
 def bnact_bwd_reduce_pair(dy1, lddy1, dy2, lddy2, csplit, u, ldu, rows, c, a, b, act):
     s1, s2 = new_stats(csplit, u.device), new_stats(c - csplit, u.device)
-    with _Timed(f"ly_bnact_bwd_reduce_kernel<{_tname(u)}, {act}>", 6.0 * rows * c, 2.0 * u.element_size() * rows * c):
+    with _Timed(f"ly_bnact_bwd_reduce_kernel<{_tname(u)}, {act}, false>", 6.0 * rows * c, 2.0 * u.element_size() * rows * c):
         capi.check(capi.lib().ly_bnact_bwd_reduce_pair(_p(dy1), lddy1, _p(dy2), lddy2, csplit, _p(u), ldu, rows, c, _p(a), _p(b), act, _p(s1), _p(s2),
                                                        capi.dtype_code(u), capi.stream_ptr()), "ly_bnact_bwd_reduce_pair")
     return s1, s2
 
 
 def bnact_bwd_apply_pair(dy1, lddy1, dy2, lddy2, csplit, u, ldu, rows, c, a, b, act, alpha, kappa, lam, du, lddu):
-    with _Timed(f"ly_bnact_bwd_apply_kernel<{_tname(u)}, {act}>", 8.0 * rows * c, 3.0 * u.element_size() * rows * c):
+    with _Timed(f"ly_bnact_bwd_apply_kernel<{_tname(u)}, {act}, false>", 8.0 * rows * c, 3.0 * u.element_size() * rows * c):
         capi.check(capi.lib().ly_bnact_bwd_apply_pair(_p(dy1), lddy1, _p(dy2), lddy2, csplit, _p(u), ldu, rows, c, _p(a), _p(b), act, _p(alpha), _p(kappa),
                                                       _p(lam), _p(du), lddu, capi.dtype_code(u), capi.stream_ptr()), "ly_bnact_bwd_apply_pair")
 
```
